# SCZwangxiao/video-ReTaKe

Measured on NVIDIA B200. Metric: 2048-frame DPSelect+PivotKV frames/s, higher is better.
Workload: dtype bf16

## Files before the change

### video-retake_b200/csrc/pivot_misc.cu

```cuda
#include <climits>

#include <stdlib.h>

#include "rtk_common.cuh"

namespace rtk {

struct RopeParams {
    int heads, L, D, n_pos, forward;
    long long stride_h, stride_l, out_stride_h, out_stride_l;
    int heads2;
    const __nv_bfloat16* x2;
    __nv_bfloat16* out2;
    long long stride_h2, stride_l2, out_stride_h2, out_stride_l2;
    int bound[6];
    float inv_scale2;
};

static bool mrope_bounds(int n_pos, const int32_t* sec, int64_t D, int bound[6]) {
    int acc = 0;
    for (int i = 0; i < 6; ++i) {
        acc += n_pos == 3 ? sec[i % 3] : 0;
        bound[i] = acc;
    }
    return n_pos != 3 || acc == D;
}

__device__ __forceinline__ int rope_pos_row(const RopeParams& p, int c) {
    if (p.n_pos == 1) return 0;
    int i = 0;
    while (i < 5 && c >= p.bound[i]) ++i;
    return i % 3;
}

__global__ void __launch_bounds__(256)
pivot_rope_table_kernel(const long long* __restrict__ pos, const float* __restrict__ inv_freq, RopeParams p, float scaling,
                        __nv_bfloat16* __restrict__ cos_t, __nv_bfloat16* __restrict__ sin_t) {
    pdl_enter();
    const int half = p.D >> 1;
    const long long total = (long long)p.L * p.D;
    for (long long i = (long long)blockIdx.x * blockDim.x + threadIdx.x; i < total; i += (long long)gridDim.x * blockDim.x) {
        const int c = (int)(i % p.D);
        const int l = (int)(i / p.D);
        const long long pv = pos[(size_t)rope_pos_row(p, c) * p.L + l];
        const float ang = inv_freq[c < half ? c : c - half] * (float)pv;
        cos_t[i] = __float2bfloat16_rn(cosf(ang) * scaling);
        sin_t[i] = __float2bfloat16_rn(sinf(ang) * scaling);
    }
}

__device__ __forceinline__ void rope_rotate_pair(float xa, float xb, float cosa, float sina, float cosb, float sinb, int forward,
                                                 float inv_scale2, __nv_bfloat16& oa, __nv_bfloat16& ob) {
    const float ta = round_bf16(xa * cosa), ra = round_bf16(-xb * sina);
    const float tb = round_bf16(xb * cosb), rb = round_bf16(xa * sinb);
    float ya, yb;
    if (forward) {
        ya = ta + ra;
        yb = tb + rb;
    } else {
        ya = round_bf16(ta - ra) * inv_scale2;
        yb = round_bf16(tb - rb) * inv_scale2;
    }
    oa = __float2bfloat16_rn(ya);
    ob = __float2bfloat16_rn(yb);
}

__device__ __forceinline__ void rope_table_entry(const RopeParams& p, const float* __restrict__ inv_freq, const long long* pv,
                                                 int c, float scaling, float& co, float& si) {
    const int half = p.D >> 1;
    const float ang = inv_freq[c < half ? c : c - half] * (float)pv[rope_pos_row(p, c)];
    co = __bfloat162float(__float2bfloat16_rn(cosf(ang) * scaling));
    si = __bfloat162float(__float2bfloat16_rn(sinf(ang) * scaling));
}

#ifndef RTK_UNROPE_TOK
#define RTK_UNROPE_TOK 2
#endif
constexpr int kUnropeTok = RTK_UNROPE_TOK;

__device__ __forceinline__ uint32_t sub_bf16x2_rn(uint32_t a, uint32_t b) {
    uint32_t d;
    asm("sub.rn.bf16x2 %0, %1, %2;" : "=r"(d) : "r"(a), "r"(b));
    return d;
}
__device__ __forceinline__ uint32_t add_bf16x2_rn(uint32_t a, uint32_t b) {
    uint32_t d;
    asm("add.rn.bf16x2 %0, %1, %2;" : "=r"(d) : "r"(a), "r"(b));
    return d;
}
__device__ __forceinline__ void unrotate_bf16x2(uint32_t xa, uint32_t xb, uint32_t cs, uint32_t sn, bool scale, float inv_scale2,
                                                uint32_t& oa, uint32_t& ob) {
    const uint32_t ta = mul_bf16x2_rn(xa, cs), ra = mul_bf16x2_rn(xb ^ 0x80008000u, sn);
    const uint32_t tb = mul_bf16x2_rn(xb, cs), rb = mul_bf16x2_rn(xa, sn);
    oa = sub_bf16x2_rn(ta, ra);
    ob = sub_bf16x2_rn(tb, rb);
    if (scale) {
        oa = scale_bf16x2_rn(oa, inv_scale2);
        ob = scale_bf16x2_rn(ob, inv_scale2);
    }
}

__device__ __forceinline__ void unrope_qk_body(const __nv_bfloat16* __restrict__ x, const long long* __restrict__ pos,
                                               const float* __restrict__ inv_freq, float scaling,
                                               __nv_bfloat16* __restrict__ out, const RopeParams& p) {
    __shared__ __align__(16) __nv_bfloat16 s_cos[kUnropeTok][128], s_sin[kUnropeTok][128];
    const int half = p.D >> 1;
    const int vec_per_row = half >> 3;
    const int ntask = (p.heads + p.heads2) * vec_per_row;
    const int tid = threadIdx.x;
    const bool scale = p.inv_scale2 != 1.0f;
    const int v0 = tid % vec_per_row, h0 = tid / vec_per_row;
    const bool second0 = h0 >= p.heads;
    const long long src_h0 = second0 ? (long long)(h0 - p.heads) * p.stride_h2 : (long long)h0 * p.stride_h;
    const long long src_l0 = second0 ? p.stride_l2 : p.stride_l;
    const __nv_bfloat16* src0 = (second0 ? p.x2 : x) + src_h0 + v0 * 8;
    for (int l0 = blockIdx.x * kUnropeTok; l0 < p.L; l0 += gridDim.x * kUnropeTok) {
        const int nl = min(kUnropeTok, p.L - l0);
        uint4 lo4[kUnropeTok], hi4[kUnropeTok];
        if (tid < ntask) {
#pragma unroll
            for (int t = 0; t < kUnropeTok; ++t) {
                if (t < nl) {
                    lo4[t] = *reinterpret_cast<const uint4*>(src0 + (l0 + t) * src_l0);
                    hi4[t] = *reinterpret_cast<const uint4*>(src0 + (l0 + t) * src_l0 + half);
                }
            }
        }
        for (int e = tid; e < nl * half; e += blockDim.x) {
            const int t = e / half, c = e - t * half;
            long long pv[3] = {0, 0, 0};
            for (int r = 0; r < p.n_pos; ++r) pv[r] = pos[(size_t)r * p.L + l0 + t];
            float co, si;
            rope_table_entry(p, inv_freq, pv, c, scaling, co, si);
            s_cos[t][c] = __float2bfloat16_rn(co);
            s_sin[t][c] = __float2bfloat16_rn(si);
        }
        __syncthreads();
#pragma unroll
        for (int t = 0; t < kUnropeTok; ++t) {
            if (t >= nl) break;
            const int l = l0 + t;
            for (int task = tid; task < ntask; task += blockDim.x) {
                const int v = task % vec_per_row, h = task / vec_per_row;
                const int c0 = v * 8;
                const bool second = h >= p.heads;
                const __nv_bfloat16* src = second ? p.x2 + (h - p.heads) * p.stride_h2 + l * p.stride_l2 : x + h * p.stride_h + l * p.stride_l;
                __nv_bfloat16* dst = second ? p.out2 + (h - p.heads) * p.out_stride_h2 + l * p.out_stride_l2
                                            : out + h * p.out_stride_h + l * p.out_stride_l;
                uint4 a4 = lo4[t], b4 = hi4[t];
                if (task != tid) {
                    a4 = *reinterpret_cast<const uint4*>(src + c0);
                    b4 = *reinterpret_cast<const uint4*>(src + c0 + half);
                }
                const uint4 cs = *reinterpret_cast<const uint4*>(&s_cos[t][c0]);
                const uint4 sn = *reinterpret_cast<const uint4*>(&s_sin[t][c0]);
                uint4 ol4, oh4;
                unrotate_bf16x2(a4.x, b4.x, cs.x, sn.x, scale, p.inv_scale2, ol4.x, oh4.x);
                unrotate_bf16x2(a4.y, b4.y, cs.y, sn.y, scale, p.inv_scale2, ol4.y, oh4.y);
                unrotate_bf16x2(a4.z, b4.z, cs.z, sn.z, scale, p.inv_scale2, ol4.z, oh4.z);
                unrotate_bf16x2(a4.w, b4.w, cs.w, sn.w, scale, p.inv_scale2, ol4.w, oh4.w);
                *reinterpret_cast<uint4*>(dst + c0) = ol4;
                *reinterpret_cast<uint4*>(dst + c0 + half) = oh4;
            }
        }
        __syncthreads();
    }
}

struct BatchLayers {
    const __nv_bfloat16* q[kMaxBatchLayers];
    const __nv_bfloat16* k[kMaxBatchLayers];
    const __nv_bfloat16* k_in[kMaxBatchLayers];
    const __nv_bfloat16* v[kMaxBatchLayers];
    __nv_bfloat16* qu[kMaxBatchLayers];
    __nv_bfloat16* ku[kMaxBatchLayers];
    const long long* pos[kMaxBatchLayers];
    const uint8_t* keymask[kMaxBatchLayers];
    __nv_bfloat16* k_out[kMaxBatchLayers];
    __nv_bfloat16* v_out[kMaxBatchLayers];
    long long* pos_out[kMaxBatchLayers];
    int32_t* keep_idx[kMaxBatchLayers];
    const __nv_bfloat16* head_scores[kMaxBatchLayers];
    long long q_stride_h[kMaxBatchLayers], q_stride_l[kMaxBatchLayers];
    long long kin_stride_h[kMaxBatchLayers], kin_stride_l[kMaxBatchLayers];
    long long k_stride_h[kMaxBatchLayers], k_stride_l[kMaxBatchLayers];
    long long v_stride_h[kMaxBatchLayers], v_stride_l[kMaxBatchLayers];
    long long out_stride_h[kMaxBatchLayers], pos_out_stride[kMaxBatchLayers];
};

__global__ void __launch_bounds__(256)
pivot_unrope_qk_batch_kernel(const __grid_constant__ BatchLayers t, const float* __restrict__ inv_freq, float scaling, RopeParams p) {
    pdl_enter();
    const int layer = blockIdx.y;
    p.stride_h = t.q_stride_h[layer]; p.stride_l = t.q_stride_l[layer];
    p.x2 = t.k_in[layer]; p.out2 = t.ku[layer];
    p.stride_h2 = t.kin_stride_h[layer]; p.stride_l2 = t.kin_stride_l[layer];
    unrope_qk_body(t.q[layer], t.pos[layer], inv_freq, scaling, t.qu[layer], p);
}

__global__ void __launch_bounds__(256)
pivot_rope_kernel(const __nv_bfloat16* __restrict__ x, const __nv_bfloat16* __restrict__ cos_t,
                  const __nv_bfloat16* __restrict__ sin_t, __nv_bfloat16* __restrict__ out, RopeParams p) {
    pdl_enter();
    const int half = p.D >> 1;
    const int vec_per_row = half >> 3;
    const long long total = (long long)(p.heads + p.heads2) * p.L * vec_per_row;
    for (long long i = (long long)blockIdx.x * blockDim.x + threadIdx.x; i < total; i += (long long)gridDim.x * blockDim.x) {
        const int v = (int)(i % vec_per_row);
        const long long hl = i / vec_per_row;
        const int l = (int)(hl % p.L);
        const int h = (int)(hl / p.L);
        const int c0 = v * 8;
        const bool second = h >= p.heads;
        const __nv_bfloat16* src = second ? p.x2 + (h - p.heads) * p.stride_h2 + l * p.stride_l2 : x + h * p.stride_h + l * p.stride_l;
        __nv_bfloat16* dst = second ? p.out2 + (h - p.heads) * p.out_stride_h2 + l * p.out_stride_l2
                                    : out + h * p.out_stride_h + l * p.out_stride_l;
        uint4 lo4 = *reinterpret_cast<const uint4*>(src + c0);
        uint4 hi4 = *reinterpret_cast<const uint4*>(src + c0 + half);
        const __nv_bfloat16* xl = reinterpret_cast<const __nv_bfloat16*>(&lo4);
        const __nv_bfloat16* xh = reinterpret_cast<const __nv_bfloat16*>(&hi4);
        uint4 ol4, oh4;
        __nv_bfloat16* ol = reinterpret_cast<__nv_bfloat16*>(&ol4);
        __nv_bfloat16* oh = reinterpret_cast<__nv_bfloat16*>(&oh4);
        const int rowa0 = rope_pos_row(p, c0), rowa1 = rope_pos_row(p, c0 + 7);
        const int rowb0 = rope_pos_row(p, c0 + half), rowb1 = rope_pos_row(p, c0 + half + 7);
        uint4 ca4, sa4, cb4, sb4;
        __nv_bfloat16* cav = reinterpret_cast<__nv_bfloat16*>(&ca4);
        __nv_bfloat16* sav = reinterpret_cast<__nv_bfloat16*>(&sa4);
        __nv_bfloat16* cbv = reinterpret_cast<__nv_bfloat16*>(&cb4);
        __nv_bfloat16* sbv = reinterpret_cast<__nv_bfloat16*>(&sb4);
        if (rowa0 == rowa1 && rowb0 == rowb1) {
            const size_t ia = ((size_t)rowa0 * p.L + l) * p.D + c0, ib = ((size_t)rowb0 * p.L + l) * p.D + c0 + half;
            ca4 = __ldg(reinterpret_cast<const uint4*>(cos_t + ia));
            sa4 = __ldg(reinterpret_cast<const uint4*>(sin_t + ia));
            cb4 = __ldg(reinterpret_cast<const uint4*>(cos_t + ib));
            sb4 = __ldg(reinterpret_cast<const uint4*>(sin_t + ib));
        } else {
#pragma unroll
            for (int e = 0; e < 8; ++e) {
                const int ca = c0 + e, cb = c0 + e + half;
                const size_t ia = ((size_t)rope_pos_row(p, ca) * p.L + l) * p.D + ca;
                const size_t ib = ((size_t)rope_pos_row(p, cb) * p.L + l) * p.D + cb;
                cav[e] = cos_t[ia]; sav[e] = sin_t[ia]; cbv[e] = cos_t[ib]; sbv[e] = sin_t[ib];
            }
        }
#pragma unroll
        for (int e = 0; e < 8; ++e)
            rope_rotate_pair(__bfloat162float(xl[e]), __bfloat162float(xh[e]), __bfloat162float(cav[e]), __bfloat162float(sav[e]),
                             __bfloat162float(cbv[e]), __bfloat162float(sbv[e]), p.forward, p.inv_scale2, ol[e], oh[e]);
        *reinterpret_cast<uint4*>(dst + c0) = ol4;
        *reinterpret_cast<uint4*>(dst + c0 + half) = oh4;
    }
}

bool key_elision_enabled();

struct KeyElide {
    const uint8_t* keymask[kMaxBatchLayers];
    int32_t* slot[kMaxBatchLayers];
    const __nv_bfloat16* k[kMaxBatchLayers];
    long long k_stride_h[kMaxBatchLayers], k_stride_l[kMaxBatchLayers];
    __nv_bfloat16* kc[kMaxBatchLayers];
    int32_t* n_keys;
    int L, KVH, D;
};

__global__ void __launch_bounds__(1024)
pivot_keymask_scan_kernel(const __grid_constant__ KeyElide e) {
    pdl_enter();
    __shared__ int wsum[32];
    const int layer = blockIdx.x, tid = threadIdx.x, lane = tid & 31, warp = tid >> 5;
    const uint8_t* __restrict__ m = e.keymask[layer];
    int32_t* __restrict__ slot = e.slot[layer];
    const int per = (e.L + 1023) / 1024;
    const int beg = min(tid * per, e.L), end = min(beg + per, e.L);
    int cnt = 0;
    for (int i = beg; i < end; ++i) cnt += !(m && m[i]);
    int inc = cnt;
#pragma unroll
    for (int o = 1; o < 32; o <<= 1) {
        const int n = __shfl_up_sync(0xffffffffu, inc, o);
        if (lane >= o) inc += n;
    }
    if (lane == 31) wsum[warp] = inc;
    __syncthreads();
    if (warp == 0) {
        const int w = wsum[lane];
        int winc = w;
#pragma unroll
        for (int o = 1; o < 32; o <<= 1) {
            const int n = __shfl_up_sync(0xffffffffu, winc, o);
            if (lane >= o) winc += n;
        }
        wsum[lane] = winc - w;
        if (lane == 31) e.n_keys[layer] = winc;
    }
    __syncthreads();
    int base = wsum[warp] + inc - cnt;
    for (int i = beg; i < end; ++i) slot[i] = (m && m[i]) ? -1 : base++;
}

__global__ void __launch_bounds__(256)
pivot_keys_compact_kernel(const __grid_constant__ KeyElide e) {
    pdl_enter();
    const int layer = blockIdx.y;
    const int vpr = e.D >> 3;
    const long long total = (long long)e.L * e.KVH * vpr;
    const int32_t* __restrict__ slot = e.slot[layer];
    for (long long i = (long long)blockIdx.x * blockDim.x + threadIdx.x; i < total; i += (long long)gridDim.x * blockDim.x) {
        const int v = (int)(i % vpr);
        const long long lh = i / vpr;
        const int h = (int)(lh % e.KVH);
        const int l = (int)(lh / e.KVH);
        const int sl = slot[l];
        if (sl < 0) continue;
        const uint4 w = __ldg(reinterpret_cast<const uint4*>(e.k[layer] + h * e.k_stride_h[layer] + l * e.k_stride_l[layer] + v * 8));
        *reinterpret_cast<uint4*>(e.kc[layer] + ((size_t)sl * e.KVH + h) * e.D + v * 8) = w;
    }
}

static int key_elide_prepare(KeyElide& ke, int n, ScoreBatch& sb, cudaStream_t st) {
    RTK_LAUNCH_PDL(pivot_keymask_scan_kernel, (unsigned)n, 1024, 0, st, ke);
    const long long total = (long long)ke.L * ke.KVH * (ke.D >> 3);
    long long gx = (total + 255) / 256;
    if (gx > 148 * 8) gx = 148 * 8;
    RTK_LAUNCH_PDL(pivot_keys_compact_kernel, dim3((unsigned)gx, (unsigned)n), 256, 0, st, ke);
    for (int i = 0; i < n; ++i) {
        sb.kc[i] = ke.kc[i];
        sb.slot[i] = ke.slot[i];
    }
    sb.n_keys = ke.n_keys;
    return 0;
}

static size_t key_elide_bytes(int64_t KVH, int64_t L, int64_t D) {
    return (((size_t)KVH * L * D * 2 + 255) & ~(size_t)255) + (((size_t)L * 4 + 255) & ~(size_t)255);
}

constexpr int kSelThreads = 1024;

__device__ void block_select_top(const uint32_t* keys, int L, int keep, int32_t* out_idx, int* sh ,
                                 int low_bit ) {
    const int tid = threadIdx.x, lane = tid & 31, warp = tid >> 5;
    const int per = (L + kSelThreads - 1) / kSelThreads;
    const int beg = min(tid * per, L), end = min(beg + per, L);
    uint32_t prefix = 0;
    for (int bit = 31; bit >= low_bit; --bit) {
        const uint32_t cand = prefix | (1u << bit);
        int cnt = 0;
        for (int i = beg; i < end; ++i) cnt += (keys[i] >= cand);
        cnt = __reduce_add_sync(0xffffffffu, cnt);
        int* buf = sh + 40 + 32 * (bit & 1);
        if (lane == 0) buf[warp] = cnt;
        __syncthreads();
        const int total = __reduce_add_sync(0xffffffffu, buf[lane]);
        if (total >= keep) prefix = cand;
    }
    __syncthreads();
    if (low_bit > 0 && (!(prefix & 0x80000000u) || (prefix >> low_bit) == (0xffffffffu >> low_bit)))
        prefix |= (1u << low_bit) - 1u;
    int gt = 0, eq = 0;
    for (int i = beg; i < end; ++i) { gt += (keys[i] > prefix); eq += (keys[i] == prefix); }
    auto block_excl_scan = [&](int v, int& total) {
        int inc = v;
#pragma unroll
        for (int o = 1; o < 32; o <<= 1) {
            const int n = __shfl_up_sync(0xffffffffu, inc, o);
            if (lane >= o) inc += n;
        }
        __syncthreads();
        if (lane == 31) sh[1 + warp] = inc;
        __syncthreads();
        if (warp == 0) {
            int w = sh[1 + lane], winc = w;
#pragma unroll
            for (int o = 1; o < 32; o <<= 1) {
                const int n = __shfl_up_sync(0xffffffffu, winc, o);
                if (lane >= o) winc += n;
            }
            sh[1 + lane] = winc - w;
            if (lane == 31) sh[33] = winc;
        }
        __syncthreads();
        total = sh[33];
        return sh[1 + warp] + inc - v;
    };
    int gt_total, eq_total;
    const int gt_before = block_excl_scan(gt, gt_total);
    const int eq_before = block_excl_scan(eq, eq_total);
    const int need = keep - gt_total;
    const int eq_taken_before = min(eq_before, need);
    int slot = gt_before + eq_taken_before;
    int eq_seen = eq_before;
    for (int i = beg; i < end; ++i) {
        const uint32_t k = keys[i];
        bool take = k > prefix;
        if (k == prefix) { take = eq_seen < need; ++eq_seen; }
        if (take) out_idx[slot++] = i;
    }
}

__device__ __forceinline__ void pivot_select_body(const __nv_bfloat16* __restrict__ head_scores, int KVH, int L,
                                                  const uint8_t* __restrict__ keymask, int keep, int32_t* __restrict__ keep_idx,
                                                  __nv_bfloat16* __restrict__ score_out, const long long* __restrict__ tpos,
                                                  long long* __restrict__ tmin_out) {
    extern __shared__ __align__(128) uint8_t smem[];
    uint32_t* keys = reinterpret_cast<uint32_t*>(smem);
    int* sh = reinterpret_cast<int*>(smem + (size_t)L * 4);
    const float rcp = 1.0f / (float)KVH;
    for (int i = threadIdx.x; i < L; i += blockDim.x) {
        float v[4] = {0.f, 0.f, 0.f, 0.f};
        for (int j = 0; j < KVH; ++j) v[j & 3] += __bfloat162float(head_scores[(size_t)j * L + i]);
        const __nv_bfloat16 s = __float2bfloat16_rn((((v[0] + v[1]) + v[2]) + v[3]) * rcp);
        if (score_out) score_out[i] = s;
        const float f = (keymask && keymask[i]) ? 1.0f : __bfloat162float(s);
        keys[i] = f32_to_ordered(f);
    }
    __syncthreads();
    block_select_top(keys, L, keep, keep_idx, sh, 16);
    if (tmin_out) {
        __syncthreads();
        long long* smin = reinterpret_cast<long long*>((reinterpret_cast<uintptr_t>(sh) + 7) & ~(uintptr_t)7);
        long long mn = LLONG_MAX;
        for (int j = threadIdx.x; j < keep; j += blockDim.x) mn = min(mn, tpos[keep_idx[j]]);
#pragma unroll
        for (int o = 16; o > 0; o >>= 1) mn = min(mn, __shfl_xor_sync(0xffffffffu, mn, o));
        if ((threadIdx.x & 31) == 0) smin[threadIdx.x >> 5] = mn;
        __syncthreads();
        if (threadIdx.x == 0) {
            for (int w = 1; w < (int)(blockDim.x >> 5); ++w) mn = min(mn, smin[w]);
            *tmin_out = mn;
        }
    }
}

__device__ __forceinline__ void st_release_sys(uint32_t* p, uint32_t v) {
    asm volatile("st.release.sys.global.u32 [%0], %1;" ::"l"(p), "r"(v) : "memory");
}
__device__ __forceinline__ uint32_t ld_acquire_sys(const uint32_t* p) {
    uint32_t v;
    asm volatile("ld.acquire.sys.global.u32 %0, [%1];" : "=r"(v) : "l"(p) : "memory");
    return v;
}
__device__ __forceinline__ unsigned long long globaltimer_ns() {
    unsigned long long t;
    asm volatile("mov.u64 %0, %%globaltimer;" : "=l"(t));
    return t;
}
__device__ __forceinline__ void xchg_wait(const uint32_t* flags, int n, uint32_t epoch, unsigned long long timeout_ns) {
    if ((int)threadIdx.x < n) {
        const unsigned long long t0 = globaltimer_ns();
        while (ld_acquire_sys(flags + threadIdx.x) != epoch) {
            __nanosleep(64);
            if (timeout_ns && globaltimer_ns() - t0 > timeout_ns) __trap();
        }
    }
    __syncthreads();
}
struct XchgPutBatch {
    const __nv_bfloat16* src[kMaxBatchLayers];
    __nv_bfloat16* dst[kMaxBatchLayers][8];
    long long n;
    int world, rank;
};
__global__ void __launch_bounds__(1024)
pivot_xchg_put_batch_kernel(const __grid_constant__ XchgPutBatch p) {
    pdl_enter();
    const int layer = blockIdx.x;
    const __nv_bfloat16* src = p.src[layer];
    for (int r = 0; r < p.world; ++r) {
        if (r == p.rank) continue;
        __nv_bfloat16* dst = p.dst[layer][r];
        if ((((uintptr_t)src | (uintptr_t)dst) & 15u) == 0) {
            const long long nv = p.n >> 3;
            for (long long i = threadIdx.x; i < nv; i += blockDim.x)
                reinterpret_cast<uint4*>(dst)[i] = reinterpret_cast<const uint4*>(src)[i];
            for (long long i = (nv << 3) + threadIdx.x; i < p.n; i += blockDim.x) dst[i] = src[i];
        } else {
            for (long long i = threadIdx.x; i < p.n; i += blockDim.x) dst[i] = src[i];
        }
    }
    __threadfence_system();
}
struct XchgFlags {
    uint32_t* flags[8];
    int world, rank;
    uint32_t epoch;
};
__global__ void __launch_bounds__(32)
pivot_xchg_flag_kernel(XchgFlags p) {
    pdl_enter();
    __threadfence_system();
    if ((int)threadIdx.x < p.world) st_release_sys(p.flags[threadIdx.x] + p.rank, p.epoch);
}

__global__ void __launch_bounds__(kSelThreads)
pivot_select_kernel(const __nv_bfloat16* __restrict__ head_scores, int KVH, int L, const uint8_t* __restrict__ keymask,
                    int keep, int32_t* __restrict__ keep_idx, __nv_bfloat16* __restrict__ score_out) {
    pdl_enter();
    pivot_select_body(head_scores, KVH, L, keymask, keep, keep_idx, score_out, nullptr, nullptr);
}

__global__ void __launch_bounds__(kSelThreads)
pivot_select_batch_kernel(const __grid_constant__ BatchLayers t, int KVH, int L, int keep, int reforge, long long* __restrict__ tmin,
                          const uint32_t* __restrict__ wait_flags, int wait_n, uint32_t wait_epoch, unsigned long long wait_ns) {
    pdl_enter();
    if (wait_flags) xchg_wait(wait_flags, wait_n, wait_epoch, wait_ns);
    const int layer = blockIdx.x;
    pivot_select_body(t.head_scores[layer], KVH, L, t.keymask[layer], keep, t.keep_idx[layer], nullptr,
                      reforge ? t.pos[layer] : nullptr, reforge ? tmin + layer : nullptr);
}

struct CompactParams {
    int KVH, L, D, keep, n_pos, reforge;
    long long stride_h, stride_l, out_stride_h;
    long long v_stride_h, v_stride_l;
    long long pos_out_stride;
    float ratio;
};

__global__ void __launch_bounds__(256)
pivot_compact_kernel(const __nv_bfloat16* __restrict__ k, const __nv_bfloat16* __restrict__ v,
                     const int32_t* __restrict__ keep_idx, __nv_bfloat16* __restrict__ k_out,
                     __nv_bfloat16* __restrict__ v_out, const long long* __restrict__ pos,
                     long long* __restrict__ pos_out, CompactParams p) {
    pdl_enter();
    if (blockIdx.x == gridDim.x - 1) {
        if (!pos) return;
        __shared__ long long smin[32];
        const int tid = threadIdx.x, lane = tid & 31, warp = tid >> 5;
        for (int r = p.reforge ? 1 : 0; r < p.n_pos; ++r)
            for (int j = tid; j < p.keep; j += blockDim.x) pos_out[(size_t)r * p.keep + j] = pos[(size_t)r * p.L + keep_idx[j]];
        if (!p.reforge) return;
        long long mn = LLONG_MAX;
        for (int j = tid; j < p.keep; j += blockDim.x) mn = min(mn, pos[keep_idx[j]]);
#pragma unroll
        for (int o = 16; o > 0; o >>= 1) mn = min(mn, __shfl_xor_sync(0xffffffffu, mn, o));
        if (lane == 0) smin[warp] = mn;
        __syncthreads();
        mn = smin[0];
        for (int w = 1; w < (int)(blockDim.x >> 5); ++w) mn = min(mn, smin[w]);
        for (int j = tid; j < p.keep; j += blockDim.x) {
            const float d = (float)(pos[keep_idx[j]] - mn);
            pos_out[j] = mn + (long long)(d * p.ratio);
        }
        return;
    }
    const int vec_per_row = p.D >> 3;
    const long long total = (long long)p.KVH * p.keep * vec_per_row;
    const long long nthreads = (long long)(gridDim.x - 1) * blockDim.x;
    for (long long i = (long long)blockIdx.x * blockDim.x + threadIdx.x; i < total; i += nthreads) {
        const int c = (int)(i % vec_per_row);
        const long long hj = i / vec_per_row;
        const int j = (int)(hj % p.keep);
        const int h = (int)(hj / p.keep);
        const int src_row = keep_idx[j];
        const size_t so = (size_t)h * p.stride_h + (size_t)src_row * p.stride_l + (size_t)c * 8;
        const size_t sv = (size_t)h * p.v_stride_h + (size_t)src_row * p.v_stride_l + (size_t)c * 8;
        const size_t dof = (size_t)h * p.out_stride_h + (size_t)j * p.D + (size_t)c * 8;
        if (k) *reinterpret_cast<uint4*>(k_out + dof) = __ldg(reinterpret_cast<const uint4*>(k + so));
        if (v) *reinterpret_cast<uint4*>(v_out + dof) = __ldg(reinterpret_cast<const uint4*>(v + sv));
    }
}

__device__ __forceinline__ void compact_rope_body(const __nv_bfloat16* __restrict__ k, const __nv_bfloat16* __restrict__ v,
                                                  const int32_t* __restrict__ keep_idx, __nv_bfloat16* __restrict__ k_out,
                                                  __nv_bfloat16* __restrict__ v_out, const long long* __restrict__ pos,
                                                  long long* __restrict__ pos_out, const long long* __restrict__ tmin,
                                                  const float* __restrict__ inv_freq, float scaling, const CompactParams& p,
                                                  const RopeParams& rp, int rotate) {
    __shared__ float s_cos[256], s_sin[256];
    __shared__ long long s_pos[3];
    const int j = blockIdx.x, tid = threadIdx.x;
    const int src_row = keep_idx[j];
    if (pos && tid < p.n_pos) {
        long long pv = pos[(size_t)tid * p.L + src_row];
        if (p.reforge && tid == 0) {
            const long long mn = *tmin;
            pv = mn + (long long)((float)(pv - mn) * p.ratio);
        }
        pos_out[(size_t)tid * p.pos_out_stride + j] = pv;
        s_pos[tid] = pv;
    }
    const int vec_per_row = p.D >> 3;
    for (int t = tid; t < p.KVH * vec_per_row; t += blockDim.x) {
        const int c = t % vec_per_row, h = t / vec_per_row;
        const size_t dof = (size_t)h * p.out_stride_h + (size_t)j * p.D + (size_t)c * 8;
        *reinterpret_cast<uint4*>(v_out + dof) =
            __ldg(reinterpret_cast<const uint4*>(v + (size_t)h * p.v_stride_h + (size_t)src_row * p.v_stride_l + (size_t)c * 8));
        if (!rotate)
            *reinterpret_cast<uint4*>(k_out + dof) =
                __ldg(reinterpret_cast<const uint4*>(k + (size_t)h * p.stride_h + (size_t)src_row * p.stride_l + (size_t)c * 8));
    }
    if (!rotate) return;
    __syncthreads();
    if (tid < p.D) rope_table_entry(rp, inv_freq, s_pos, tid, scaling, s_cos[tid], s_sin[tid]);
    __syncthreads();
    const int half = p.D >> 1, hv = half >> 3;
    for (int t = tid; t < p.KVH * hv; t += blockDim.x) {
        const int c0 = (t % hv) * 8, h = t / hv;
        const __nv_bfloat16* src = k + (size_t)h * p.stride_h + (size_t)src_row * p.stride_l;
        __nv_bfloat16* dst = k_out + (size_t)h * p.out_stride_h + (size_t)j * p.D;
        uint4 lo4 = *reinterpret_cast<const uint4*>(src + c0);
        uint4 hi4 = *reinterpret_cast<const uint4*>(src + c0 + half);
        const __nv_bfloat16* xl = reinterpret_cast<const __nv_bfloat16*>(&lo4);
        const __nv_bfloat16* xh = reinterpret_cast<const __nv_bfloat16*>(&hi4);
        uint4 ol4, oh4;
        __nv_bfloat16* ol = reinterpret_cast<__nv_bfloat16*>(&ol4);
        __nv_bfloat16* oh = reinterpret_cast<__nv_bfloat16*>(&oh4);
#pragma unroll
        for (int e = 0; e < 8; ++e)
            rope_rotate_pair(__bfloat162float(xl[e]), __bfloat162float(xh[e]), s_cos[c0 + e], s_sin[c0 + e], s_cos[c0 + half + e],
                             s_sin[c0 + half + e], 1, 1.0f, ol[e], oh[e]);
        *reinterpret_cast<uint4*>(dst + c0) = ol4;
        *reinterpret_cast<uint4*>(dst + c0 + half) = oh4;
    }
}

__global__ void __launch_bounds__(128)
pivot_compact_rope_batch_kernel(const __grid_constant__ BatchLayers t, const long long* __restrict__ tmin,
                                const float* __restrict__ inv_freq, float scaling, CompactParams p, RopeParams rp, int rotate) {
    pdl_enter();
    const int layer = blockIdx.y;
    p.stride_h = t.k_stride_h[layer]; p.stride_l = t.k_stride_l[layer];
    p.v_stride_h = t.v_stride_h[layer]; p.v_stride_l = t.v_stride_l[layer];
    p.out_stride_h = t.out_stride_h[layer];
    p.pos_out_stride = t.pos_out_stride[layer];
    compact_rope_body(t.k[layer], t.v[layer], t.keep_idx[layer], t.k_out[layer], t.v_out[layer], t.pos[layer], t.pos_out[layer],
                      tmin + layer, inv_freq, scaling, p, rp, rotate);
}

struct CopyJobs {
    int n;
    const __nv_bfloat16* src[4];
    __nv_bfloat16* dst[4];
    int heads[4], rows[4];
    long long src_stride_h[4], src_stride_l[4], dst_stride_h[4], dst_stride_l[4];
    long long vec_end[4];
    int D;
};

__global__ void __launch_bounds__(256)
kv_block_copy_kernel(CopyJobs j) {
    pdl_enter();
    const int vpr = j.D >> 3;
    const long long total = j.vec_end[j.n - 1];
    for (long long i = (long long)blockIdx.x * blockDim.x + threadIdx.x; i < total; i += (long long)gridDim.x * blockDim.x) {
        int k = 0;
        while (i >= j.vec_end[k]) ++k;
        const long long li = i - (k ? j.vec_end[k - 1] : 0);
        const int c = (int)(li % vpr);
        const long long hr = li / vpr;
        const int r = (int)(hr % j.rows[k]);
        const int h = (int)(hr / j.rows[k]);
        const uint4 v = __ldg(reinterpret_cast<const uint4*>(j.src[k] + h * j.src_stride_h[k] + r * j.src_stride_l[k] + c * 8));
        *reinterpret_cast<uint4*>(j.dst[k] + h * j.dst_stride_h[k] + r * j.dst_stride_l[k] + c * 8) = v;
    }
}

long long g_launches = 0;
static int g_key_elision = -1;
bool key_elision_enabled() {
    if (g_key_elision < 0) {
        const char* e = getenv("RTK_NO_KEY_ELISION");
        g_key_elision = (e && e[0] == '1') ? 0 : 1;
    }
    return g_key_elision != 0;
}
unsigned long long xchg_timeout_ns() {
    static const unsigned long long ns = [] {
        const char* e = getenv("RTK_XCHG_TIMEOUT_S");
        const double s = (e && e[0]) ? atof(e) : 120.0;
        return s > 0.0 ? (unsigned long long)(s * 1e9) : 0ull;
    }();
    return ns;
}
bool pdl_enabled() {
    static const bool on = [] {
        const char* e = getenv("RTK_NO_PDL");
        return !(e && e[0] && e[0] != '0');
    }();
    return on;
}

}

using namespace rtk;

extern "C" int rtk_version(void) { return RTK_ABI_VERSION; }

extern "C" int rtk_debug_key_elision(int on) {
    const int prev = rtk::key_elision_enabled() ? 1 : 0;
    if (on >= 0) rtk::g_key_elision = on ? 1 : 0;
    return prev;
}

#ifndef RTK_BUILD_ID
#define RTK_BUILD_ID "unknown"
#endif
extern "C" const char* rtk_build_id(void) { return RTK_BUILD_ID; }

extern "C" int64_t rtk_launch_count(void) { return (int64_t)rtk::g_launches; }

extern "C" const char* rtk_error_string(int code) {
    if (code == 0) return "ok";
    if (code > 0) return cudaGetErrorString((cudaError_t)code);
    switch (code) {
        case RTK_E_BADARG: return "rtk: bad argument (null pointer or non-positive size)";
        case RTK_E_ALIGN: return "rtk: pointer or stride not 16-byte aligned";
        case RTK_E_UNSUPPORTED: return "rtk: shape outside the supported envelope";
        case RTK_E_WORKSPACE: return "rtk: workspace too small";
        case RTK_E_DRIVER: return "rtk: cuTensorMapEncodeTiled unavailable or failed";
        default: return "rtk: unknown error";
    }
}

static int rope_launch(const void* x, const void* cos, const void* sin, void* out, const RopeParams& p, cudaStream_t st) {
    const long long total = (long long)(p.heads + p.heads2) * p.L * (p.D / 16);
    long long grid = (total + 255) / 256;
    if (grid > 148 * 16) grid = 148 * 16;
    RTK_LAUNCH_PDL(pivot_rope_kernel, (unsigned)grid, 256, 0, st, (const __nv_bfloat16*)x, (const __nv_bfloat16*)cos, (const __nv_bfloat16*)sin, (__nv_bfloat16*)out, p);
    return 0;
}

extern "C" int rtk_pivot_rope(const void* x, int64_t heads, int64_t L, int64_t D, int64_t stride_h, int64_t stride_l,
                              const void* cos, const void* sin, int n_pos, const int32_t* mrope_section_host,
                              float inv_scale2, int forward, void* out, int64_t out_stride_h, int64_t out_stride_l,
                              void* stream) {
    RTK_NVTX("rtk_pivot_rope");
    if (!x || !cos || !sin || !out || heads < 1 || L < 1 || D < 16) return RTK_E_BADARG;
    if (D % 16 != 0 || (n_pos != 1 && n_pos != 3)) return RTK_E_UNSUPPORTED;
    if (n_pos == 3 && !mrope_section_host) return RTK_E_BADARG;
    if ((((uintptr_t)x | (uintptr_t)out) & 15u) != 0) return RTK_E_ALIGN;
    if ((stride_h | stride_l | out_stride_h | out_stride_l) % 8 != 0) return RTK_E_ALIGN;
    RopeParams p;
    p.heads = (int)heads; p.L = (int)L; p.D = (int)D; p.n_pos = n_pos; p.forward = forward;
    p.stride_h = stride_h; p.stride_l = stride_l; p.out_stride_h = out_stride_h; p.out_stride_l = out_stride_l;
    p.inv_scale2 = inv_scale2;
    p.heads2 = 0; p.x2 = nullptr; p.out2 = nullptr;
    p.stride_h2 = p.stride_l2 = p.out_stride_h2 = p.out_stride_l2 = 0;
    if (!mrope_bounds(n_pos, mrope_section_host, D, p.bound)) return RTK_E_UNSUPPORTED;
    return rope_launch(x, cos, sin, out, p, (cudaStream_t)stream);
}

extern "C" int rtk_pivot_select(const void* head_scores, int64_t KVH, int64_t L, const uint8_t* keymask, int64_t keep,
                                int32_t* keep_idx, void* score_out, void* stream) {
    RTK_NVTX("rtk_pivot_select");
    if (!head_scores || !keep_idx || KVH < 1 || L < 1 || keep < 1 || keep > L) return RTK_E_BADARG;
    if (L > 16384) return RTK_E_UNSUPPORTED;
    const size_t smem = (size_t)L * 4 + 112 * 4;
    cudaError_t e = cudaFuncSetAttribute(pivot_select_kernel, cudaFuncAttributeMaxDynamicSharedMemorySize, (int)smem);
    if (e != cudaSuccess) return (int)e;
    RTK_LAUNCH_PDL(pivot_select_kernel, 1, kSelThreads, smem, (cudaStream_t)stream, (const __nv_bfloat16*)head_scores, (int)KVH,
                   (int)L, keymask, (int)keep, keep_idx, (__nv_bfloat16*)score_out);
    return 0;
}

extern "C" int rtk_pivot_compact(const void* k, const void* v, int64_t KVH, int64_t L, int64_t D, int64_t stride_h,
                                 int64_t stride_l, const int32_t* keep_idx, int64_t keep, void* k_out, void* v_out,
                                 int64_t out_stride_h, const int64_t* pos, int n_pos, int64_t* pos_out, int reforge,
                                 void* stream) {
    RTK_NVTX("rtk_pivot_compact");
    if ((!k && !v) || !keep_idx || (k && !k_out) || (v && !v_out) || KVH < 1 || L < 1 || D < 8 || keep < 1 || keep > L)
        return RTK_E_BADARG;
    if (pos && (!pos_out || n_pos < 1)) return RTK_E_BADARG;
    if (D % 8 != 0) return RTK_E_UNSUPPORTED;
    if ((((uintptr_t)k | (uintptr_t)v | (uintptr_t)k_out | (uintptr_t)v_out) & 15u) != 0) return RTK_E_ALIGN;
    if ((stride_h | stride_l | out_stride_h) % 8 != 0) return RTK_E_ALIGN;
    CompactParams p;
    p.KVH = (int)KVH; p.L = (int)L; p.D = (int)D; p.keep = (int)keep; p.n_pos = n_pos; p.reforge = reforge;
    p.stride_h = stride_h; p.stride_l = stride_l; p.out_stride_h = out_stride_h;
    p.v_stride_h = stride_h; p.v_stride_l = stride_l;
    p.pos_out_stride = keep;
    p.ratio = (float)((double)keep / (double)L);
    const long long total = KVH * keep * (D / 8);
    long long grid = (total + 255) / 256;
    if (grid > 148 * 8) grid = 148 * 8;
    RTK_LAUNCH_PDL(pivot_compact_kernel, (unsigned)(grid + 1), 256, 0, (cudaStream_t)stream,  (const __nv_bfloat16*)k, (const __nv_bfloat16*)v, keep_idx, (__nv_bfloat16*)k_out, (__nv_bfloat16*)v_out, (const long long*)pos, (long long*)pos_out, p);
    return 0;
}

extern "C" int rtk_pivot_rope_tables(const int64_t* pos, int n_pos, int64_t L, int64_t D, const float* inv_freq,
                                     const int32_t* mrope_section_host, float attention_scaling, void* cos_out,
                                     void* sin_out, void* stream) {
    RTK_NVTX("rtk_pivot_rope_tables");
    if (!pos || !inv_freq || !cos_out || !sin_out || L < 1 || D < 2) return RTK_E_BADARG;
    if (D % 2 != 0 || (n_pos != 1 && n_pos != 3)) return RTK_E_UNSUPPORTED;
    if (n_pos == 3 && !mrope_section_host) return RTK_E_BADARG;
    RopeParams p;
    p.heads = 1; p.L = (int)L; p.D = (int)D; p.n_pos = n_pos; p.forward = 0;
    p.stride_h = p.stride_l = p.out_stride_h = p.out_stride_l = 0;
    p.heads2 = 0; p.x2 = nullptr; p.out2 = nullptr;
    p.stride_h2 = p.stride_l2 = p.out_stride_h2 = p.out_stride_l2 = 0;
    p.inv_scale2 = 1.0f;
    if (!mrope_bounds(n_pos, mrope_section_host, D, p.bound)) return RTK_E_UNSUPPORTED;
    long long grid = (L * D + 255) / 256;
    if (grid > 148 * 8) grid = 148 * 8;
    RTK_LAUNCH_PDL(pivot_rope_table_kernel, (unsigned)grid, 256, 0, (cudaStream_t)stream,  (const long long*)pos, inv_freq, p, attention_scaling, (__nv_bfloat16*)cos_out, (__nv_bfloat16*)sin_out);
    return 0;
}

static size_t align256(size_t x) { return (x + 255) & ~(size_t)255; }

extern "C" size_t rtk_pivot_update_batch_workspace_bytes(int64_t H, int64_t KVH, int64_t L, int64_t D, int64_t n_layers) {
    if (H < 1 || KVH < 1 || L < 1 || D < 1 || n_layers < 1) return 0;
    const size_t n = (size_t)(n_layers < kMaxBatchLayers ? n_layers : kMaxBatchLayers);
    return align256(rtk_pivot_score_workspace_bytes(H * (int64_t)n, L)) +
           n * (align256((size_t)H * L * D * 2) + align256((size_t)KVH * L * D * 2)) + align256(n * sizeof(long long)) + 256 +
           n * key_elide_bytes(KVH, L, D) + 256;
}

extern "C" size_t rtk_pivot_update_workspace_bytes(int64_t H, int64_t KVH, int64_t L, int64_t D) {
    return rtk_pivot_update_batch_workspace_bytes(H, KVH, L, D, 1);
}

#ifndef RTK_UNROT_TOKEN_MAJOR
#define RTK_UNROT_TOKEN_MAJOR 1
#endif

static int pivot_update_group(const rtk_pivot_update_args* a, int n, char* ws, cudaStream_t st) {
    const rtk_pivot_update_args& a0 = a[0];
    const int64_t H = a0.H, KVH = a0.KVH, L = a0.L, D = a0.D;
    const bool reforge = a0.reforge != 0;
    const int64_t uq_sh = RTK_UNROT_TOKEN_MAJOR ? D : L * D, uq_sl = RTK_UNROT_TOKEN_MAJOR ? H * D : D;
    const int64_t uk_sh = RTK_UNROT_TOKEN_MAJOR ? D : L * D, uk_sl = RTK_UNROT_TOKEN_MAJOR ? KVH * D : D;
    void* score_ws = ws;                ws += align256(rtk_pivot_score_workspace_bytes(H * n, L));
    char* qu0 = ws;                     ws += (size_t)n * align256((size_t)H * L * D * 2);
    char* ku0 = ws;                     ws += (size_t)n * align256((size_t)KVH * L * D * 2);
    long long* tmin = (long long*)ws;   ws += align256((size_t)n * sizeof(long long)) + 256;
    char* kc0 = ws;                     ws += (size_t)n * align256((size_t)KVH * L * D * 2);
    char* slot0 = ws;                   ws += (size_t)n * align256((size_t)L * 4);
    int32_t* nkeys_ws = (int32_t*)ws;

    BatchLayers t = {};
    ScoreBatch sb = {};
    sb.n = n; sb.H = H; sb.KVH = KVH; sb.L = L; sb.D = D;
    for (int i = 0; i < kMaxBatchLayers; ++i) {
        const rtk_pivot_update_args& x = a[i < n ? i : 0];
        char* qu = qu0 + (size_t)(i < n ? i : 0) * align256((size_t)H * L * D * 2);
        char* ku = ku0 + (size_t)(i < n ? i : 0) * align256((size_t)KVH * L * D * 2);
        t.q[i] = (const __nv_bfloat16*)x.q;       t.q_stride_h[i] = x.q_stride_h;     t.q_stride_l[i] = x.q_stride_l;
        t.k_in[i] = (const __nv_bfloat16*)x.k;    t.kin_stride_h[i] = x.k_stride_h;   t.kin_stride_l[i] = x.k_stride_l;
        t.qu[i] = (__nv_bfloat16*)qu;             t.ku[i] = (__nv_bfloat16*)ku;
        t.k[i] = reforge ? (const __nv_bfloat16*)ku : (const __nv_bfloat16*)x.k;
        t.k_stride_h[i] = reforge ? uk_sh : x.k_stride_h;
        t.k_stride_l[i] = reforge ? uk_sl : x.k_stride_l;
        t.v[i] = (const __nv_bfloat16*)x.v;       t.v_stride_h[i] = x.v_stride_h;     t.v_stride_l[i] = x.v_stride_l;
        t.pos[i] = (const long long*)x.pos;       t.keymask[i] = x.keymask;
        t.k_out[i] = (__nv_bfloat16*)x.k_out;     t.v_out[i] = (__nv_bfloat16*)x.v_out;
        t.out_stride_h[i] = x.out_stride_h;
        t.pos_out[i] = (long long*)x.pos_out;     t.pos_out_stride[i] = x.pos_out_stride > 0 ? x.pos_out_stride : x.keep;
        t.keep_idx[i] = x.keep_idx;               t.head_scores[i] = (const __nv_bfloat16*)x.head_scores;
        if (i < n) {
            sb.q[i] = reforge ? (const void*)qu : x.q;
            sb.k[i] = reforge ? (const void*)ku : x.k;
            sb.q_stride_h[i] = reforge ? uq_sh : x.q_stride_h;   sb.q_stride_l[i] = reforge ? uq_sl : x.q_stride_l;
            sb.k_stride_h[i] = reforge ? uk_sh : x.k_stride_h;   sb.k_stride_l[i] = reforge ? uk_sl : x.k_stride_l;
            sb.head_scores[i] = x.head_scores;
        }
    }
    RopeParams rp = {};
    rp.heads = (int)H; rp.L = (int)L; rp.D = (int)D; rp.n_pos = a0.n_pos; rp.forward = 0;
    rp.out_stride_h = uq_sh; rp.out_stride_l = uq_sl;
    rp.heads2 = (int)KVH; rp.out_stride_h2 = uk_sh; rp.out_stride_l2 = uk_sl;
    rp.inv_scale2 = a0.inv_scale2;
    mrope_bounds(a0.n_pos, a0.mrope_section, D, rp.bound);
    const bool xchg = a0.xchg_world > 1;
    const int64_t score_rows = a0.score_rows > 0 ? a0.score_rows : KVH;
    if (reforge && !a0.skip_score) {
        if (a0.inv_freq) {
            RTK_LAUNCH_PDL(pivot_unrope_qk_batch_kernel, dim3((unsigned)((L + kUnropeTok - 1) / kUnropeTok), (unsigned)n), 256, 0, st, t, a0.inv_freq,
                           a0.attention_scaling, rp);
        } else {
            rp.stride_h = a0.q_stride_h; rp.stride_l = a0.q_stride_l;
            rp.x2 = t.k_in[0]; rp.out2 = t.ku[0]; rp.stride_h2 = a0.k_stride_h; rp.stride_l2 = a0.k_stride_l;
            const int rc = rope_launch(a0.q, a0.cos, a0.sin, t.qu[0], rp, st);
            if (rc) return rc;
        }
    }
    if (!a0.skip_score) {
        bool any_mask = false;
        for (int i = 0; i < n; ++i) any_mask = any_mask || a[i].keymask != nullptr;
        if (any_mask && key_elision_enabled()) {
            KeyElide ke = {};
            ke.L = (int)L; ke.KVH = (int)KVH; ke.D = (int)D; ke.n_keys = nkeys_ws;
            for (int i = 0; i < kMaxBatchLayers; ++i) {
                const int j = i < n ? i : 0;
                ke.keymask[i] = a[j].keymask;
                ke.slot[i] = (int32_t*)(slot0 + (size_t)j * align256((size_t)L * 4));
                ke.k[i] = t.k[j]; ke.k_stride_h[i] = t.k_stride_h[j]; ke.k_stride_l[i] = t.k_stride_l[j];
                ke.kc[i] = (__nv_bfloat16*)(kc0 + (size_t)j * align256((size_t)KVH * L * D * 2));
            }
            int rc = key_elide_prepare(ke, n, sb, st);
            if (rc) return rc;
        }
        if (a0.ev_score_begin) cudaEventRecord((cudaEvent_t)a0.ev_score_begin, st);
        int rc = pivot_score_batch(sb, score_ws, rtk_pivot_score_workspace_bytes(H * n, L), st);
        if (rc) return rc;
        if (a0.ev_score_end) cudaEventRecord((cudaEvent_t)a0.ev_score_end, st);
    }
    if (a0.skip_select) {
        if (xchg) {
            XchgPutBatch xp = {};
            xp.n = (long long)KVH * L; xp.world = a0.xchg_world; xp.rank = a0.xchg_rank;
            for (int i = 0; i < n; ++i) {
                xp.src[i] = (const __nv_bfloat16*)a[i].head_scores;
                for (int r = 0; r < a0.xchg_world; ++r)
                    xp.dst[i][r] = (__nv_bfloat16*)a[i].xchg_scores[r] + (size_t)a0.xchg_rank * KVH * L;
            }
            RTK_LAUNCH_PDL(pivot_xchg_put_batch_kernel, (unsigned)n, 1024, 0, st, xp);
            XchgFlags xf = {};
            xf.world = a0.xchg_world; xf.rank = a0.xchg_rank; xf.epoch = a0.xchg_epoch;
            for (int r = 0; r < a0.xchg_world; ++r) xf.flags[r] = a0.xchg_flags[r];
            RTK_LAUNCH_PDL(pivot_xchg_flag_kernel, 1, 32, 0, st, xf);
        }
        return 0;
    }
    {
        const size_t smem = (size_t)L * 4 + 112 * 4;
        cudaError_t e = cudaFuncSetAttribute(pivot_select_batch_kernel, cudaFuncAttributeMaxDynamicSharedMemorySize, (int)smem);
        if (e != cudaSuccess) return (int)e;
        RTK_LAUNCH_PDL(pivot_select_batch_kernel, (unsigned)n, kSelThreads, smem, st, t, (int)score_rows, (int)L, (int)a0.keep,
                       reforge ? 1 : 0, tmin, (const uint32_t*)(xchg ? a0.xchg_flags[a0.xchg_rank] : nullptr),
                       xchg ? a0.xchg_world : 0, a0.xchg_epoch, xchg_timeout_ns());
    }
    {
        CompactParams p = {};
        p.KVH = (int)KVH; p.L = (int)L; p.D = (int)D; p.keep = (int)a0.keep; p.n_pos = a0.pos ? a0.n_pos : 0; p.reforge = a0.reforge;
        p.ratio = (float)((double)a0.keep / (double)L);
        RopeParams rq = {};
        rq.D = (int)D; rq.n_pos = a0.n_pos; rq.L = (int)a0.keep;
        for (int i = 0; i < 6; ++i) rq.bound[i] = rp.bound[i];
        RTK_LAUNCH_PDL(pivot_compact_rope_batch_kernel, dim3((unsigned)a0.keep, (unsigned)n), 128, 0, st, t, (const long long*)tmin,
                       a0.inv_freq, a0.attention_scaling, p, rq, (reforge && a0.inv_freq) ? 1 : 0);
    }
    return 0;
}

static int update_check(const rtk_pivot_update_args* layers, int64_t n, const void* workspace, size_t workspace_bytes) {
    if (!layers || n < 1 || !workspace) return RTK_E_BADARG;
    const rtk_pivot_update_args& a0 = layers[0];
    const bool scores = !a0.skip_score, selects = !a0.skip_select, xchg = a0.xchg_world > 1;
    if (!scores && !selects) return RTK_E_BADARG;
    if (a0.H < 1 || a0.KVH < 1 || a0.L < 1 || (selects && (a0.keep < 1 || a0.keep > a0.L))) return RTK_E_BADARG;
    if (a0.L > 16384 || a0.D % 16 != 0 || a0.D > 256) return RTK_E_UNSUPPORTED;
    if (scores && ((a0.D != 64 && a0.D != 128) || a0.H % a0.KVH != 0 || a0.H > 256)) return RTK_E_UNSUPPORTED;
    if (xchg) {
        if (n > kMaxBatchLayers) return RTK_E_UNSUPPORTED;
        if (a0.xchg_world > 8 || a0.xchg_rank < 0 || a0.xchg_rank >= a0.xchg_world || (scores && selects)) return RTK_E_BADARG;
    }
    if (a0.reforge && !a0.inv_freq && n > 1) return RTK_E_UNSUPPORTED;
    int bound[6];
    if (a0.reforge && (scores || a0.inv_freq) && !mrope_bounds(a0.n_pos, a0.mrope_section, a0.D, bound)) return RTK_E_UNSUPPORTED;
    if (((uintptr_t)workspace & 255u) != 0) return RTK_E_ALIGN;
    if (workspace_bytes < rtk_pivot_update_batch_workspace_bytes(a0.H, a0.KVH, a0.L, a0.D, n)) return RTK_E_WORKSPACE;
    for (int64_t i = 0; i < n; ++i) {
        const rtk_pivot_update_args& x = layers[i];
        if (!x.q || !x.k || !x.v || !x.k_out || !x.v_out || !x.keep_idx || !x.head_scores) return RTK_E_BADARG;
        if (x.H != a0.H || x.KVH != a0.KVH || x.L != a0.L || x.D != a0.D || x.keep != a0.keep || x.reforge != a0.reforge ||
            x.n_pos != a0.n_pos || x.inv_freq != a0.inv_freq || x.attention_scaling != a0.attention_scaling ||
            x.inv_scale2 != a0.inv_scale2 || x.skip_select != a0.skip_select || x.skip_score != a0.skip_score ||
            x.score_rows != a0.score_rows || x.xchg_world != a0.xchg_world || x.xchg_rank != a0.xchg_rank ||
            x.xchg_epoch != a0.xchg_epoch || (x.pos == nullptr) != (a0.pos == nullptr))
            return RTK_E_UNSUPPORTED;
        for (int j = 0; j < 3; ++j)
            if (x.mrope_section[j] != a0.mrope_section[j]) return RTK_E_UNSUPPORTED;
        if (x.reforge && (!x.pos || !x.pos_out || (!x.inv_freq && (!x.cos || !x.sin)))) return RTK_E_BADARG;
        if (xchg) {
            for (int r = 0; r < a0.xchg_world; ++r)
                if (!x.xchg_scores[r] || !a0.xchg_flags[r]) return RTK_E_BADARG;
            const char* own = (const char*)x.xchg_scores[a0.xchg_rank];
            if (a0.skip_score && (const char*)x.head_scores != own) return RTK_E_BADARG;
            if (a0.skip_select && (const char*)x.head_scores != own + (size_t)a0.xchg_rank * a0.KVH * a0.L * 2) return RTK_E_BADARG;
        }
        if (x.pos && (selects || x.reforge) && (!x.pos_out || x.n_pos < 1 || x.n_pos > 3)) return RTK_E_BADARG;
        uintptr_t ptrs = 0;
        int64_t strides = 0;
        if (scores) {
            ptrs |= (uintptr_t)x.q;
            strides |= x.q_stride_h | x.q_stride_l;
        }
        if (scores || !x.reforge) {
            ptrs |= (uintptr_t)x.k;
            strides |= x.k_stride_h | x.k_stride_l;
        }
        if (selects) {
            ptrs |= (uintptr_t)x.v | (uintptr_t)x.k_out | (uintptr_t)x.v_out;
            strides |= x.v_stride_h | x.v_stride_l | x.out_stride_h;
        }
        if ((ptrs & 15u) != 0 || strides % 8 != 0) return RTK_E_ALIGN;
    }
    return 0;
}

extern "C" int rtk_pivot_update(const rtk_pivot_update_args* a, void* stream) {
    RTK_NVTX("rtk_pivot_update");
    if (!a) return RTK_E_BADARG;
    const int rc = update_check(a, 1, a->workspace, a->workspace_bytes);
    if (rc) return rc;
    return pivot_update_group(a, 1, (char*)a->workspace, (cudaStream_t)stream);
}

extern "C" int rtk_pivot_update_batch(const rtk_pivot_update_args* layers, int64_t n_layers, void* workspace,
                                      size_t workspace_bytes, void* stream) {
    RTK_NVTX("rtk_pivot_update_batch");
    int rc = update_check(layers, n_layers, workspace, workspace_bytes);
    if (rc) return rc;
    for (int64_t i = 0; i < n_layers; i += kMaxBatchLayers) {
        const int n = (int)((n_layers - i) < kMaxBatchLayers ? (n_layers - i) : kMaxBatchLayers);
        rc = pivot_update_group(layers + i, n, (char*)workspace, (cudaStream_t)stream);
        if (rc) return rc;
    }
    return 0;
}

extern "C" int rtk_kv_block_copy(int n_jobs, const void* const* src, void* const* dst, const int64_t* heads, const int64_t* rows,
                                 const int64_t* src_stride_h, const int64_t* src_stride_l, const int64_t* dst_stride_h,
                                 const int64_t* dst_stride_l, int64_t D, void* stream) {
    RTK_NVTX("rtk_kv_block_copy");
    if (n_jobs < 1 || n_jobs > 4 || !src || !dst || !heads || !rows || D < 8) return RTK_E_BADARG;
    if (D % 8 != 0) return RTK_E_UNSUPPORTED;
    CopyJobs j;
    j.n = n_jobs;
    j.D = (int)D;
    long long acc = 0;
    for (int k = 0; k < n_jobs; ++k) {
        if (!src[k] || !dst[k] || heads[k] < 1 || rows[k] < 0) return RTK_E_BADARG;
        if ((((uintptr_t)src[k] | (uintptr_t)dst[k]) & 15u) != 0) return RTK_E_ALIGN;
        if ((src_stride_h[k] | src_stride_l[k] | dst_stride_h[k] | dst_stride_l[k]) % 8 != 0) return RTK_E_ALIGN;
        j.src[k] = (const __nv_bfloat16*)src[k];
        j.dst[k] = (__nv_bfloat16*)dst[k];
        j.heads[k] = (int)heads[k];
        j.rows[k] = (int)rows[k];
        j.src_stride_h[k] = src_stride_h[k]; j.src_stride_l[k] = src_stride_l[k];
        j.dst_stride_h[k] = dst_stride_h[k]; j.dst_stride_l[k] = dst_stride_l[k];
        acc += heads[k] * rows[k] * (D / 8);
        j.vec_end[k] = acc;
    }
    for (int k = n_jobs; k < 4; ++k) j.vec_end[k] = acc;
    if (acc == 0) return 0;
    long long grid = (acc + 255) / 256;
    if (grid > 148 * 8) grid = 148 * 8;
    RTK_LAUNCH_PDL(kv_block_copy_kernel, (unsigned)grid, 256, 0, (cudaStream_t)stream, j);
    return 0;
}
```

### video-retake_b200/csrc/pivot_score.cu

```cuda
#include <cuda.h>

#include "rtk_common.cuh"

namespace rtk {

constexpr int kTile = 128;
constexpr int kHeadDim = 128;
constexpr int kPair = 2;
constexpr int kStages = 2;
constexpr int kASlots = 2;
constexpr int kAccBufs = 4;
constexpr int kStatSlots = kStages + kAccBufs;
constexpr uint32_t kTileBytes = kTile * kHeadDim * 2;
constexpr uint32_t kHalfBytes = kTile * 64 * 2;

struct ScoreSmem {
    static constexpr uint32_t a_tile = 0;
    static constexpr uint32_t b_ring = kASlots * kPair * kTileBytes;
    static constexpr uint32_t stats = b_ring + kStages * kTileBytes;
    static constexpr uint32_t merge = stats + kStatSlots * kTile * 4;
    static constexpr uint32_t bars = merge + 4 * kTile * 2 * 4;
    static constexpr uint32_t n_bars = 4 + 2 * kStages + 2 * kAccBufs + kStatSlots;
    static constexpr uint32_t tmem_ptr = bars + n_bars * 8;
    static constexpr uint32_t total = tmem_ptr + 16;
};

__device__ __forceinline__ void tmem_alloc(uint32_t smem_dst, uint32_t ncols) {
    asm volatile("tcgen05.alloc.cta_group::1.sync.aligned.shared::cta.b32 [%0], %1;" ::"r"(smem_dst), "r"(ncols) : "memory");
    asm volatile("tcgen05.relinquish_alloc_permit.cta_group::1.sync.aligned;" ::: "memory");
}
__device__ __forceinline__ void tmem_dealloc(uint32_t taddr, uint32_t ncols) {
    asm volatile("tcgen05.dealloc.cta_group::1.sync.aligned.b32 %0, %1;" ::"r"(taddr), "r"(ncols) : "memory");
}
__device__ __forceinline__ void tc_fence_before() { asm volatile("tcgen05.fence::before_thread_sync;" ::: "memory"); }
__device__ __forceinline__ void tc_fence_after() { asm volatile("tcgen05.fence::after_thread_sync;" ::: "memory"); }
__device__ __forceinline__ void tc_commit(uint32_t bar) {
    asm volatile("tcgen05.commit.cta_group::1.mbarrier::arrive::one.shared::cluster.b64 [%0];" ::"r"(bar) : "memory");
}
__device__ __forceinline__ void umma_bf16(uint32_t tmem_d, uint64_t adesc, uint64_t bdesc, uint32_t idesc, uint32_t accum) {
    asm volatile(
        "{\n\t.reg .pred p;\n\t"
        "setp.ne.b32 p, %4, 0;\n\t"
        "tcgen05.mma.cta_group::1.kind::f16 [%0], %1, %2, %3, p;\n\t}"
        ::"r"(tmem_d), "l"(adesc), "l"(bdesc), "r"(idesc), "r"(accum)
        : "memory");
}
__device__ __forceinline__ void tmem_ld_wait() { asm volatile("tcgen05.wait::ld.sync.aligned;" ::: "memory"); }
__device__ __forceinline__ void tmem_ld64(uint32_t taddr, uint32_t (&r)[64]) {
    asm volatile(
        "tcgen05.ld.sync.aligned.32x32b.x64.b32 "
        "{%0, %1, %2, %3, %4, %5, %6, %7, %8, %9, %10, %11, %12, %13, %14, %15, "
        "%16, %17, %18, %19, %20, %21, %22, %23, %24, %25, %26, %27, %28, %29, %30, %31, "
        "%32, %33, %34, %35, %36, %37, %38, %39, %40, %41, %42, %43, %44, %45, %46, %47, "
        "%48, %49, %50, %51, %52, %53, %54, %55, %56, %57, %58, %59, %60, %61, %62, %63}, [%64];"
        : "=r"(r[0]), "=r"(r[1]), "=r"(r[2]), "=r"(r[3]), "=r"(r[4]), "=r"(r[5]), "=r"(r[6]), "=r"(r[7]),
          "=r"(r[8]), "=r"(r[9]), "=r"(r[10]), "=r"(r[11]), "=r"(r[12]), "=r"(r[13]), "=r"(r[14]), "=r"(r[15]),
          "=r"(r[16]), "=r"(r[17]), "=r"(r[18]), "=r"(r[19]), "=r"(r[20]), "=r"(r[21]), "=r"(r[22]), "=r"(r[23]),
          "=r"(r[24]), "=r"(r[25]), "=r"(r[26]), "=r"(r[27]), "=r"(r[28]), "=r"(r[29]), "=r"(r[30]), "=r"(r[31]),
          "=r"(r[32]), "=r"(r[33]), "=r"(r[34]), "=r"(r[35]), "=r"(r[36]), "=r"(r[37]), "=r"(r[38]), "=r"(r[39]),
          "=r"(r[40]), "=r"(r[41]), "=r"(r[42]), "=r"(r[43]), "=r"(r[44]), "=r"(r[45]), "=r"(r[46]), "=r"(r[47]),
          "=r"(r[48]), "=r"(r[49]), "=r"(r[50]), "=r"(r[51]), "=r"(r[52]), "=r"(r[53]), "=r"(r[54]), "=r"(r[55]),
          "=r"(r[56]), "=r"(r[57]), "=r"(r[58]), "=r"(r[59]), "=r"(r[60]), "=r"(r[61]), "=r"(r[62]), "=r"(r[63])
        : "r"(taddr)
        : "memory");
}
__device__ __forceinline__ void add_bf16_pair(float& acc_lo, float& acc_hi, uint32_t packed) {
    asm("{\n\t.reg .b16 lo, hi;\n\t"
        "mov.b32 {lo, hi}, %2;\n\t"
        "add.rn.f32.bf16 %0, lo, %0;\n\t"
        "add.rn.f32.bf16 %1, hi, %1;\n\t}"
        : "+f"(acc_lo), "+f"(acc_hi)
        : "r"(packed));
}

__device__ __forceinline__ void tma_load_3d(uint32_t dst, const CUtensorMap* map, int c0, int c1, int c2, uint32_t bar) {
    asm volatile(
        "cp.async.bulk.tensor.3d.shared::cluster.global.tile.mbarrier::complete_tx::bytes [%0], [%1, {%3, %4, %5}], [%2];"
        ::"r"(dst), "l"(reinterpret_cast<uint64_t>(map)), "r"(bar), "r"(c0), "r"(c1), "r"(c2)
        : "memory");
}
__device__ __forceinline__ float ex2f(float x) {
    float y;
    asm("ex2.approx.ftz.f32 %0, %1;" : "=f"(y) : "f"(x));
    return y;
}
__device__ __forceinline__ float lg2f(float x) {
    float y;
    asm("lg2.approx.ftz.f32 %0, %1;" : "=f"(y) : "f"(x));
    return y;
}

__device__ __forceinline__ uint64_t umma_desc_sw128(uint32_t smem_addr) {
    return (uint64_t)((smem_addr & 0x3ffffu) >> 4) | ((uint64_t)1 << 16) | ((uint64_t)(1024 >> 4) << 32) |
           ((uint64_t)1 << 46) | ((uint64_t)2 << 61);
}
constexpr uint32_t kIdesc = (1u << 4) | (1u << 7) | (1u << 10) | ((uint32_t)(kTile >> 3) << 17) | ((uint32_t)(kTile >> 4) << 24);

template <int NL>
struct ScoreMaps {
    CUtensorMap q[NL], k[NL];
    CUtensorMap kc[NL];
};

struct ScoreParams {
    int H, G, L, nt;
    int Hl;
    int n_atoms;
    int q_dim1_is_l, k_dim1_is_l;
    float inv_sqrt_d;
    const int32_t* n_keys;
    int kc_dim1_is_l;
    float2* ml_part;
    float* stats;
    float* colsum_part;
};

constexpr float kLog2e = 1.4426950408889634f;

__device__ __forceinline__ uint64_t pk2(float lo, float hi) {
    uint64_t d;
    asm("mov.b64 %0, {%1, %2};" : "=l"(d) : "f"(lo), "f"(hi));
    return d;
}
__device__ __forceinline__ void upk2(uint64_t v, float& lo, float& hi) {
    asm("mov.b64 {%0, %1}, %2;" : "=f"(lo), "=f"(hi) : "l"(v));
}
__device__ __forceinline__ uint64_t mul2(uint64_t a, uint64_t b) {
    uint64_t d;
    asm("mul.rn.f32x2 %0, %1, %2;" : "=l"(d) : "l"(a), "l"(b));
    return d;
}
__device__ __forceinline__ uint64_t fma2(uint64_t a, uint64_t b, uint64_t c) {
    uint64_t d;
    asm("fma.rn.f32x2 %0, %1, %2, %3;" : "=l"(d) : "l"(a), "l"(b), "l"(c));
    return d;
}
__device__ __forceinline__ uint64_t add2(uint64_t a, uint64_t b) {
    uint64_t d;
    asm("add.rn.f32x2 %0, %1, %2;" : "=l"(d) : "l"(a), "l"(b));
    return d;
}

__device__ __forceinline__ void mbar_wait_feeder(uint32_t bar, uint32_t parity) {
    while (!mbar_try_wait(bar, parity)) {
    }
}

__device__ __forceinline__ float round_bf16_inplace(float a) {
    uint32_t d;
    asm("cvt.rn.bf16x2.f32 %0, %1, %2;" : "=r"(d) : "f"(a), "f"(0.f));
    return __uint_as_float(d);
}

__device__ __forceinline__ uint64_t logit_chain2(uint32_t r0, uint32_t r1, uint64_t inv2) {
    float t0, t1;
    upk2(mul2(pk2(round_bf16_inplace(__uint_as_float(r0)), round_bf16_inplace(__uint_as_float(r1))), inv2), t0, t1);
    return pk2(round_bf16_inplace(t0), round_bf16_inplace(t1));
}
__device__ __forceinline__ float logit_chain1(float acc, float inv) { return round_bf16(round_bf16(acc) * inv); }

__device__ __forceinline__ uint64_t ex2_mufu2(uint64_t x2) {
    float x0, x1;
    upk2(x2, x0, x1);
    return pk2(ex2f(x0), ex2f(x1));
}

struct SoftmaxState {
    float m = -INFINITY;
    uint64_t acc = 0;
    float c0 = 0.f, c1 = 0.f;
};

template <int PASS>
__device__ __forceinline__ void softmax_cols(uint32_t (&r)[64], int valid, SoftmaxState& st, const float* cq, float inv,
                                             uint64_t inv2, uint64_t l2e2) {
    constexpr int NC = 64;
    if (PASS == 1) {
        if (valid < NC) {
#pragma unroll
            for (int i = 0; i < NC; ++i)
                if (i >= valid) r[i] = 0xff800000u;
        }
        float mx = fmaxf(fmaxf(__uint_as_float(r[0]), __uint_as_float(r[1])), __uint_as_float(r[2]));
#pragma unroll
        for (int i = 3; i < NC - 1; i += 2) mx = fmaxf(fmaxf(mx, __uint_as_float(r[i])), __uint_as_float(r[i + 1]));
        mx = fmaxf(mx, __uint_as_float(r[NC - 1]));
        const float mn = fmaxf(st.m, logit_chain1(mx, inv));
        if (!(mn > -INFINITY)) return;
        const float mm = mn * kLog2e;
        const float sc = ex2f(fmaf(st.m, kLog2e, -mm));
        st.acc = mul2(st.acc, pk2(sc, sc));
        st.m = mn;
        const uint64_t nmm = pk2(-mm, -mm);
#pragma unroll
        for (int i = 0; i < NC; i += 4) {
            st.acc = add2(st.acc, ex2_mufu2(fma2(logit_chain2(r[i], r[i + 1], inv2), l2e2, nmm)));
            st.acc = add2(st.acc, ex2_mufu2(fma2(logit_chain2(r[i + 2], r[i + 3], inv2), l2e2, nmm)));
        }
    } else {
#pragma unroll
        for (int i = 0; i < NC; i += 4) {
            const float4 cc = *reinterpret_cast<const float4*>(cq + i);
            float e0, e1, e2, e3;
            upk2(ex2_mufu2(fma2(logit_chain2(r[i], r[i + 1], inv2), l2e2, pk2(-cc.x, -cc.y))), e0, e1);
            upk2(ex2_mufu2(fma2(logit_chain2(r[i + 2], r[i + 3], inv2), l2e2, pk2(-cc.z, -cc.w))), e2, e3);
            add_bf16_pair(st.c0, st.c1, pack_bf16x2_rn(e0, e1));
            add_bf16_pair(st.c0, st.c1, pack_bf16x2_rn(e2, e3));
        }
    }
}

struct TileRange {
    int g, g1, Gl;
    int nt;
    int nt_a, nta;
    int layer, n_layers, Hl, geff;
    const int32_t* n_keys;
    __device__ __forceinline__ void set_layer_range() {
        nt_a = n_keys ? (n_keys[layer] + kTile - 1) / kTile : nt;
        nta = (nt_a + kPair - 1) / kPair;
        Gl = Hl * nta * nt;
        int ge = Gl / ((nt + 1) / 2);
        ge = ge < 1 ? 1 : (ge > (int)gridDim.x ? (int)gridDim.x : ge);
        geff = ge;
        if ((int)blockIdx.x < geff) {
            g = (int)((unsigned)Gl * blockIdx.x / (unsigned)geff);
            g1 = (int)((unsigned)Gl * (blockIdx.x + 1) / (unsigned)geff);
        } else {
            g = g1 = 0;
        }
    }
    __device__ __forceinline__ bool next_cta_reaches_end_of(int ul) const {
        return (int)((unsigned)Gl * (blockIdx.x + 2) / (unsigned)geff) >= (ul + 1) * nt;
    }
    __device__ __forceinline__ TileRange(int H, int Hl_, int nt_, const int32_t* n_keys_) : nt(nt_), layer(0), Hl(Hl_), n_keys(n_keys_) {
        n_layers = H / Hl_;
        set_layer_range();
    }
    __device__ __forceinline__ bool next(int& ul, int& tb0, int& tb1) {
        while (g >= g1) {
            if (++layer >= n_layers) return false;
            set_layer_range();
        }
        ul = g / nt;
        tb0 = g - ul * nt;
        const int left = g1 - g;
        tb1 = (left < nt - tb0) ? tb0 + left : nt;
        g += tb1 - tb0;
        return true;
    }
};

constexpr int kGroups = 4;
constexpr int kSoftmaxWarps = 4 * kGroups;
constexpr int kScoreThreads2 = (2 + kSoftmaxWarps) * 32;
constexpr int kTileArrivals = 8;

template <int PASS, int NL>
__global__ void __launch_bounds__(kScoreThreads2, 1)
pivot_score_kernel(const __grid_constant__ ScoreMaps<NL> maps, ScoreParams prm) {
    if (RTK_PDL_EARLY_SCORE) pdl_trigger();
    extern __shared__ __align__(1024) uint8_t smem_raw[];
    const uint32_t base = (smem_u32(smem_raw) + 1023u) & ~1023u;
    uint8_t* smem = smem_raw + (base - smem_u32(smem_raw));
    const int warp = threadIdx.x >> 5, lane = threadIdx.x & 31;

    const uint32_t bar0 = base + ScoreSmem::bars;
    auto a_full = [&](int i) { return bar0 + 8 * i; };
    auto a_empty = [&](int i) { return bar0 + 16 + 8 * i; };
    auto b_full = [&](int s) { return bar0 + 32 + 8 * s; };
    auto b_empty = [&](int s) { return bar0 + 32 + 8 * (kStages + s); };
    auto t_full = [&](int b) { return bar0 + 32 + 8 * (2 * kStages + b); };
    auto t_empty = [&](int b) { return bar0 + 32 + 8 * (2 * kStages + kAccBufs + b); };
    auto st_full = [&](int i) { return bar0 + 32 + 8 * (2 * kStages + 2 * kAccBufs + i); };

    if (threadIdx.x == 0) {
        for (int i = 0; i < 2; ++i) { mbar_init(a_full(i), 1); mbar_init(a_empty(i), 1); }
        for (int s = 0; s < kStages; ++s) { mbar_init(b_full(s), 1); mbar_init(b_empty(s), 1); }
        for (int b = 0; b < kAccBufs; ++b) { mbar_init(t_full(b), 1); mbar_init(t_empty(b), kTileArrivals); }
        for (int i = 0; i < kStatSlots; ++i) mbar_init(st_full(i), 1);
        fence_mbar_init();
    }
    if (warp == 1) tmem_alloc(base + ScoreSmem::tmem_ptr, 512);
    tc_fence_before();
    __syncthreads();
    tc_fence_after();
    pdl_wait();
    const uint32_t tmem_base = *reinterpret_cast<volatile uint32_t*>(smem + ScoreSmem::tmem_ptr);

    const int nt = prm.nt;
    const size_t hl = (size_t)prm.H * nt * kTile;
    const bool elide = (PASS == 2) && prm.n_keys != nullptr;
    const CUtensorMap* a_maps = (PASS == 1) ? maps.q : (elide ? maps.kc : maps.k);
    const CUtensorMap* b_maps = (PASS == 1) ? maps.k : maps.q;
    const int a_l1 = (PASS == 1) ? prm.q_dim1_is_l : (elide ? prm.kc_dim1_is_l : prm.k_dim1_is_l);
    const int b_l1 = (PASS == 1) ? prm.k_dim1_is_l : prm.q_dim1_is_l;
    TileRange range(prm.H, prm.Hl, nt, elide ? prm.n_keys : nullptr);
    int ul, tb0, tb1;

    if (warp == 0) {
        if (lane == 0) {
            uint32_t cnt = 0, ucnt = 0;
            while (range.next(ul, tb0, tb1)) {
                const int layer = range.layer;
                const int h = ul / range.nta, ta = (ul - h * range.nta) * kPair;
                const int hh = layer * prm.Hl + h;
                const int nt_a = range.nt_a;
                const CUtensorMap* a_map = a_maps + layer;
                const CUtensorMap* b_map = b_maps + layer;
                const int a_head = (PASS == 1) ? h : h / prm.G;
                const int b_head = (PASS == 1) ? h / prm.G : h;
                const int as = ucnt % kASlots;
                mbar_wait_feeder(a_empty(as), ((ucnt / kASlots) & 1u) ^ 1u);
                mbar_arrive_expect_tx(a_full(as), kPair * prm.n_atoms * kHalfBytes);
                for (int pa = 0; pa < kPair; ++pa)
                    for (int kk = 0; kk < prm.n_atoms; ++kk) {
                        const int row = ((ta + pa < nt_a) ? ta + pa : ta) * kTile;
                        tma_load_3d(base + ScoreSmem::a_tile + (as * kPair + pa) * kTileBytes + kk * kHalfBytes, a_map, kk * 64,
                                    a_l1 ? row : a_head, a_l1 ? a_head : row, a_full(as));
                    }
                ++ucnt;
                for (int tb = tb0; tb < tb1; ++tb, ++cnt) {
                    const int s = cnt % kStages;
                    mbar_wait_feeder(b_empty(s), ((cnt / kStages) & 1u) ^ 1u);
                    mbar_arrive_expect_tx(b_full(s), prm.n_atoms * kHalfBytes);
                    const uint32_t dst = base + ScoreSmem::b_ring + s * kTileBytes;
                    for (int kk = 0; kk < prm.n_atoms; ++kk) {
                        const int row = tb * kTile;
                        tma_load_3d(dst + kk * kHalfBytes, b_map, kk * 64, b_l1 ? row : b_head, b_l1 ? b_head : row,
                                    b_full(s));
                    }
                    if (PASS == 2) {
                        const int sl = cnt % kStatSlots;
                        mbar_arrive_expect_tx(st_full(sl), kTile * 4u);
                        bulk_g2s(base + ScoreSmem::stats + sl * kTile * 4u,
                                 prm.stats + (size_t)hh * nt * kTile + (size_t)tb * kTile, kTile * 4u, st_full(sl));
                    }
                }
            }
        }
    } else if (warp == 1) {
        uint32_t cnt = 0, ucnt = 0;
        while (range.next(ul, tb0, tb1)) {
            const int as = ucnt % kASlots;
            mbar_wait_feeder(a_full(as), (ucnt / kASlots) & 1u);
            ++ucnt;
            for (int tb = tb0; tb < tb1; ++tb, ++cnt) {
                const int s = cnt % kStages, bp = 2 * (int)(cnt & 1u);
                mbar_wait_feeder(b_full(s), (cnt / kStages) & 1u);
                mbar_wait_feeder(t_empty(bp), ((cnt >> 1) & 1u) ^ 1u);
                mbar_wait_feeder(t_empty(bp + 1), ((cnt >> 1) & 1u) ^ 1u);
                tc_fence_after();
                if (elect_one()) {
                    const uint32_t b0 = base + ScoreSmem::b_ring + s * kTileBytes;
                    const int nks = prm.n_atoms * 4;
#pragma unroll
                    for (int pa = 0; pa < 2; ++pa) {
                        const uint32_t a0 = base + ScoreSmem::a_tile + (as * 2 + pa) * kTileBytes;
#pragma unroll 8
                        for (int ks = 0; ks < nks; ++ks) {
                            const uint32_t off = (ks >> 2) * kHalfBytes + (ks & 3) * 32;
                            umma_bf16(tmem_base + (bp + pa) * kTile, umma_desc_sw128(a0 + off), umma_desc_sw128(b0 + off), kIdesc,
                                      ks > 0 ? 1u : 0u);
                        }
                        tc_commit(t_full(bp + pa));
                    }
                    tc_commit(b_empty(s));
                    if (tb == tb1 - 1) tc_commit(a_empty(as));
                }
                __syncwarp();
            }
        }
    } else {
        const int sw = warp - 2;
        const int grp = sw >> 2;
        const int quarter = warp & 3;
        const int row = quarter * 32 + lane;
        const int half = grp & 1;
        const uint32_t lane_addr = tmem_base + ((uint32_t)(quarter * 32) << 16) + half * 64;
        float* merge = reinterpret_cast<float*>(smem + ScoreSmem::merge);
        const float inv = prm.inv_sqrt_d;
        const uint64_t inv2 = pk2(inv, inv), l2e2 = pk2(kLog2e, kLog2e);
        uint32_t cnt = 0;
        while (range.next(ul, tb0, tb1)) {
            const int hl_ = ul / range.nta, ta = (ul - hl_ * range.nta) * 2 + (grp >> 1);
            const int h = range.layer * prm.Hl + hl_;
            const bool has_tile = ta < range.nt_a;
            SoftmaxState st;
            for (int tb = tb0; tb < tb1; ++tb, ++cnt) {
                const int b = 2 * (int)(cnt & 1u) + (grp >> 1);
                mbar_wait(t_full(b), (cnt >> 1) & 1u);
                tc_fence_after();
                if (PASS == 2) mbar_wait(st_full(cnt % kStatSlots), (cnt / kStatSlots) & 1u);
                const int valid = prm.L - tb * kTile - half * 64;
                const float* cq = reinterpret_cast<const float*>(smem + ScoreSmem::stats) + (cnt % kStatSlots) * kTile + half * 64;
                if (has_tile) {
                    uint32_t r[64];
                    tmem_ld64(lane_addr + b * kTile, r);
                    tmem_ld_wait();
                    softmax_cols<PASS>(r, valid, st, cq, inv, inv2, l2e2);
                }
                tc_fence_before();
                __syncwarp();
                if (lane == 0) mbar_arrive(t_empty(b));
            }
            const float m = st.m;
            float a0, a1;
            upk2(st.acc, a0, a1);
            if (PASS == 2) { a0 = st.c0; a1 = st.c1; }
            const bool first = (tb0 == 0), last = (tb1 == nt);
            const int part = first ? 0 : (last ? 2 : 1);
            const bool fill1 = first && (last || range.next_cta_reaches_end_of(ul)), fill2 = first && last;
            const size_t o = (size_t)h * nt * kTile + (size_t)ta * kTile + row;
            const int g_lo = grp & ~1;
            const bool folder = (grp == g_lo) && has_tile;
            if (PASS == 1) {
                merge[(grp * kTile + row) * 2] = m;
                merge[(grp * kTile + row) * 2 + 1] = a0 + a1;
                asm volatile("bar.sync 1, %0;" ::"n"(kSoftmaxWarps * 32) : "memory");
                if (folder) {
                    float mn = -INFINITY;
                    for (int g = g_lo; g < g_lo + 2; ++g) mn = fmaxf(mn, merge[(g * kTile + row) * 2]);
                    float lt = 0.f;
                    for (int g = g_lo; g < g_lo + 2; ++g) {
                        const float mg = merge[(g * kTile + row) * 2];
                        if (mg > -INFINITY) lt += merge[(g * kTile + row) * 2 + 1] * ex2f((mg - mn) * kLog2e);
                    }
                    prm.ml_part[(size_t)part * hl + o] = make_float2(mn, lt);
                    if (fill1) prm.ml_part[hl + o] = make_float2(-INFINITY, 0.f);
                    if (fill2) prm.ml_part[2 * hl + o] = make_float2(-INFINITY, 0.f);
                }
                asm volatile("bar.sync 1, %0;" ::"n"(kSoftmaxWarps * 32) : "memory");
            } else {
                merge[grp * kTile + row] = a0 + a1;
                asm volatile("bar.sync 1, %0;" ::"n"(kSoftmaxWarps * 32) : "memory");
                if (folder) {
                    const float cs = merge[g_lo * kTile + row] + merge[(g_lo + 1) * kTile + row];
                    prm.colsum_part[(size_t)part * hl + o] = cs;
                    if (fill1) prm.colsum_part[hl + o] = 0.f;
                    if (fill2) prm.colsum_part[2 * hl + o] = 0.f;
                }
                asm volatile("bar.sync 1, %0;" ::"n"(kSoftmaxWarps * 32) : "memory");
            }
        }
    }
    tc_fence_before();
    __syncthreads();
    if (warp == 1) tmem_dealloc(tmem_base, 512);
}

__global__ void pivot_stats_merge_kernel(const float2* __restrict__ ml_part, int H, int L, int Lpad, float* __restrict__ stats) {
    pdl_enter();
    const int q = blockIdx.x * blockDim.x + threadIdx.x;
    const int h = blockIdx.y;
    if (q >= Lpad) return;
    const size_t o = (size_t)h * Lpad + q, hl = (size_t)H * Lpad;
    const float2 p0 = ml_part[o], p1 = ml_part[hl + o], p2 = ml_part[2 * hl + o];
    const float mn = fmaxf(fmaxf(p0.x, p1.x), p2.x);
    float lt = 0.f;
    if (p0.x > -INFINITY) lt += p0.y * ex2f((p0.x - mn) * kLog2e);
    if (p1.x > -INFINITY) lt += p1.y * ex2f((p1.x - mn) * kLog2e);
    if (p2.x > -INFINITY) lt += p2.y * ex2f((p2.x - mn) * kLog2e);
    stats[o] = (q < L) ? fmaf(mn, kLog2e, lg2f(lt)) : INFINITY;
}

struct HeadScoreOut {
    __nv_bfloat16* p[kMaxBatchLayers];
    const int32_t* slot[kMaxBatchLayers];
    int KVH;
};

__global__ void pivot_head_reduce_kernel(const float* __restrict__ colsum_part, int H, int G, int L, int Lpad,
                                         const __grid_constant__ HeadScoreOut out) {
    pdl_enter();
    const int k = blockIdx.x * blockDim.x + threadIdx.x;
    const int g = blockIdx.y;
    if (k >= L) return;
    const size_t hl = (size_t)H * Lpad;
    const int layer = g / out.KVH;
    int col = k;
    if (out.slot[layer]) {
        col = out.slot[layer][k];
        if (col < 0) {
            out.p[layer][(size_t)(g - layer * out.KVH) * L + k] = __float2bfloat16_rn(1.0f);
            return;
        }
    }
    float v[4] = {0.f, 0.f, 0.f, 0.f};
    for (int j = 0; j < G; ++j) {
        const size_t o = (size_t)(g * G + j) * Lpad + col;
        v[j & 3] += round_bf16((colsum_part[o] + colsum_part[hl + o]) + colsum_part[2 * hl + o]);
    }
    const float s = ((v[0] + v[1]) + v[2]) + v[3];
    out.p[layer][(size_t)(g - layer * out.KVH) * L + k] = __float2bfloat16_rn(s * (1.0f / (float)G));
}

typedef CUresult (*EncodeTiledFn)(CUtensorMap*, CUtensorMapDataType, cuuint32_t, void*, const cuuint64_t*, const cuuint64_t*,
                                  const cuuint32_t*, const cuuint32_t*, CUtensorMapInterleave, CUtensorMapSwizzle,
                                  CUtensorMapL2promotion, CUtensorMapFloatOOBfill);

static EncodeTiledFn get_encode_fn() {
    static EncodeTiledFn fn = nullptr;
    if (fn) return fn;
    void* p = nullptr;
    cudaDriverEntryPointQueryResult qres;
    if (cudaGetDriverEntryPoint("cuTensorMapEncodeTiled", &p, cudaEnableDefault, &qres) != cudaSuccess ||
        qres != cudaDriverEntryPointSuccess)
        return nullptr;
    fn = reinterpret_cast<EncodeTiledFn>(p);
    return fn;
}

static int make_map(CUtensorMap* map, const void* ptr, int64_t heads, int64_t L, int64_t D, int64_t stride_h,
                    int64_t stride_l, int* dim1_is_l) {
    EncodeTiledFn enc = get_encode_fn();
    if (!enc) return RTK_E_DRIVER;
    const bool l_first = (heads == 1) || (stride_l <= stride_h);
    *dim1_is_l = l_first ? 1 : 0;
    cuuint64_t dims[3] = {(cuuint64_t)D, (cuuint64_t)(l_first ? L : heads), (cuuint64_t)(l_first ? heads : L)};
    cuuint64_t strides[2] = {(cuuint64_t)((l_first ? stride_l : stride_h) * 2), (cuuint64_t)((l_first ? stride_h : stride_l) * 2)};
    if (heads == 1) strides[1] = (cuuint64_t)(stride_l * 2) * (cuuint64_t)L;
    cuuint32_t box[3] = {64u, (cuuint32_t)(l_first ? kTile : 1), (cuuint32_t)(l_first ? 1 : kTile)};
    cuuint32_t estr[3] = {1u, 1u, 1u};
    CUresult r = enc(map, CU_TENSOR_MAP_DATA_TYPE_BFLOAT16, 3, const_cast<void*>(ptr), dims, strides, box, estr,
                     CU_TENSOR_MAP_INTERLEAVE_NONE, CU_TENSOR_MAP_SWIZZLE_128B, CU_TENSOR_MAP_L2_PROMOTION_L2_256B,
                     CU_TENSOR_MAP_FLOAT_OOB_FILL_NONE);
    return r == CUDA_SUCCESS ? 0 : RTK_E_DRIVER;
}

}

using namespace rtk;

extern "C" size_t rtk_pivot_score_workspace_bytes(int64_t H, int64_t L) {
    if (H < 1 || L < 1) return 0;
    const size_t lpad = (size_t)((L + kTile - 1) / kTile) * kTile;
    return 10 * (size_t)H * lpad * sizeof(float);
}

namespace rtk {

template <int NL>
static int score_launch(const ScoreBatch& b, ScoreParams prm, cudaStream_t st) {
    ScoreMaps<NL> maps;
    for (int l = 0; l < b.n; ++l) {
        int ql = 0, kl = 0;
        int rc = make_map(&maps.q[l], b.q[l], b.H, b.L, b.D, b.q_stride_h[l], b.q_stride_l[l], &ql);
        if (rc) return rc;
        rc = make_map(&maps.k[l], b.k[l], b.KVH, b.L, b.D, b.k_stride_h[l], b.k_stride_l[l], &kl);
        if (rc) return rc;
        if (l == 0) { prm.q_dim1_is_l = ql; prm.k_dim1_is_l = kl; }
        else if (ql != prm.q_dim1_is_l || kl != prm.k_dim1_is_l) return RTK_E_UNSUPPORTED;
        if (prm.n_keys) {
            int cl = 0;
            rc = make_map(&maps.kc[l], b.kc[l], b.KVH, b.L, b.D, b.D, b.KVH * b.D, &cl);
            if (rc) return rc;
            prm.kc_dim1_is_l = cl;
        } else {
            maps.kc[l] = maps.k[l];
        }
    }
    for (int l = b.n; l < NL; ++l) { maps.q[l] = maps.q[0]; maps.k[l] = maps.k[0]; maps.kc[l] = maps.kc[0]; }
    int dev = 0, sms = 0;
    cudaGetDevice(&dev);
    cudaDeviceGetAttribute(&sms, cudaDevAttrMultiProcessorCount, dev);
    const int units = prm.Hl * ((prm.nt + kPair - 1) / kPair);
    const long long gmax = (long long)units * prm.nt / ((prm.nt + 1) / 2);
    const int grid = (int)(gmax < sms ? (gmax < 1 ? 1 : gmax) : sms);
    const size_t smem = ScoreSmem::total + 1024;
    cudaError_t e = cudaFuncSetAttribute(pivot_score_kernel<1, NL>, cudaFuncAttributeMaxDynamicSharedMemorySize, (int)smem);
    if (e != cudaSuccess) return (int)e;
    e = cudaFuncSetAttribute(pivot_score_kernel<2, NL>, cudaFuncAttributeMaxDynamicSharedMemorySize, (int)smem);
    if (e != cudaSuccess) return (int)e;
    HeadScoreOut out;
    out.KVH = (int)b.KVH;
    for (int l = 0; l < kMaxBatchLayers; ++l) {
        out.p[l] = reinterpret_cast<__nv_bfloat16*>(b.head_scores[l < b.n ? l : 0]);
        out.slot[l] = prm.n_keys ? b.slot[l < b.n ? l : 0] : nullptr;
    }
    RTK_LAUNCH_PDL((pivot_score_kernel<1, NL>), grid, kScoreThreads2, smem, st, maps, prm);
    dim3 g1((unsigned)((prm.nt * kTile + 255) / 256), (unsigned)prm.H);
    RTK_LAUNCH_PDL(pivot_stats_merge_kernel, g1, 256, 0, st, prm.ml_part, prm.H, prm.L, prm.nt * kTile, prm.stats);
    RTK_LAUNCH_PDL((pivot_score_kernel<2, NL>), grid, kScoreThreads2, smem, st, maps, prm);
    dim3 g2((unsigned)((prm.L + 255) / 256), (unsigned)(b.KVH * b.n));
    RTK_LAUNCH_PDL(pivot_head_reduce_kernel, g2, 256, 0, st, prm.colsum_part, prm.H, prm.G, prm.L, prm.nt * kTile, out);
    return 0;
}

int pivot_score_batch(const ScoreBatch& b, void* workspace, size_t workspace_bytes, cudaStream_t st) {
    if (b.n < 1 || b.n > kMaxBatchLayers || !workspace || b.H < 1 || b.KVH < 1 || b.L < 1) return RTK_E_BADARG;
    if ((b.D != 64 && b.D != 128) || b.H % b.KVH != 0 || b.L > 16384 || b.H > 256) return RTK_E_UNSUPPORTED;
    if (((uintptr_t)workspace & 15u) != 0) return RTK_E_ALIGN;
    for (int l = 0; l < b.n; ++l) {
        if (!b.q[l] || !b.k[l] || !b.head_scores[l]) return RTK_E_BADARG;
        if ((((uintptr_t)b.q[l] | (uintptr_t)b.k[l]) & 15u) != 0) return RTK_E_ALIGN;
        if ((b.q_stride_h[l] | b.q_stride_l[l] | b.k_stride_h[l] | b.k_stride_l[l]) % 8 != 0) return RTK_E_ALIGN;
    }
    if (workspace_bytes < rtk_pivot_score_workspace_bytes(b.H * b.n, b.L)) return RTK_E_WORKSPACE;

    ScoreParams prm;
    prm.H = (int)(b.H * b.n);
    prm.Hl = (int)b.H;
    prm.G = (int)(b.H / b.KVH);
    prm.L = (int)b.L;
    prm.nt = (int)((b.L + kTile - 1) / kTile);
    prm.n_atoms = (int)(b.D / 64);
    prm.q_dim1_is_l = prm.k_dim1_is_l = prm.kc_dim1_is_l = 0;
    prm.n_keys = b.n_keys;
    if (b.n_keys)
        for (int l = 0; l < b.n; ++l)
            if (!b.kc[l] || !b.slot[l] || ((uintptr_t)b.kc[l] & 15u) != 0) return RTK_E_BADARG;
    const float sq = (float)sqrt((double)b.D);
    prm.inv_sqrt_d = 1.0f / sq;
    const size_t plane = (size_t)prm.H * prm.nt * kTile;
    prm.ml_part = reinterpret_cast<float2*>(workspace);
    prm.stats = reinterpret_cast<float*>(workspace) + 6 * plane;
    prm.colsum_part = prm.stats + plane;
    return b.n == 1 ? score_launch<1>(b, prm, st) : score_launch<kMaxBatchLayers>(b, prm, st);
}

}

extern "C" int rtk_pivot_score(const void* q, int64_t H, int64_t q_stride_h, int64_t q_stride_l, const void* k, int64_t KVH,
                               int64_t k_stride_h, int64_t k_stride_l, int64_t L, int64_t D, void* head_scores,
                               void* workspace, size_t workspace_bytes, void* stream) {
    RTK_NVTX("rtk_pivot_score");
    if (!q || !k || !head_scores || !workspace || H < 1 || KVH < 1 || L < 1) return RTK_E_BADARG;
    ScoreBatch b = {};
    b.n = 1; b.H = H; b.KVH = KVH; b.L = L; b.D = D;
    b.q[0] = q; b.k[0] = k; b.head_scores[0] = head_scores;
    b.q_stride_h[0] = q_stride_h; b.q_stride_l[0] = q_stride_l; b.k_stride_h[0] = k_stride_h; b.k_stride_l[0] = k_stride_l;
    return pivot_score_batch(b, workspace, workspace_bytes, (cudaStream_t)stream);
}
```

### video-retake_b200/csrc/rtk_common.cuh

```cuda
#pragma once

#include <cuda_bf16.h>
#include <cuda_runtime.h>
#include <nvtx3/nvToolsExt.h>
#include <stdint.h>

#include "../../include/rtk_b200.h"

namespace rtk {

extern long long g_launches;

#define RTK_CHECK_LAUNCH()                                   \
    do {                                                     \
        ++::rtk::g_launches;                                 \
        cudaError_t e__ = cudaGetLastError();                \
        if (e__ != cudaSuccess) return (int)e__;             \
    } while (0)

constexpr int kWarp = 32;

struct NvtxRange {
    explicit NvtxRange(const char* name) { nvtxRangePushA(name); }
    ~NvtxRange() { nvtxRangePop(); }
    NvtxRange(const NvtxRange&) = delete;
    NvtxRange& operator=(const NvtxRange&) = delete;
};
#define RTK_NVTX(name) ::rtk::NvtxRange nvtx_range__(name)

struct DisAux {
    float* sim;
    float* nrm;
    long long si, sp;
};
int dpselect_sim_nrm(const void* x, int64_t T, int64_t N, int64_t C, DisAux aux, cudaStream_t st);

constexpr int kMaxBatchLayers = 32;
struct ScoreBatch {
    int n;
    int64_t H, KVH, L, D;
    const void* q[kMaxBatchLayers];
    const void* k[kMaxBatchLayers];
    void* head_scores[kMaxBatchLayers];
    int64_t q_stride_h[kMaxBatchLayers], q_stride_l[kMaxBatchLayers], k_stride_h[kMaxBatchLayers], k_stride_l[kMaxBatchLayers];
    const void* kc[kMaxBatchLayers];
    const int32_t* slot[kMaxBatchLayers];
    const int32_t* n_keys;
};
int pivot_score_batch(const ScoreBatch& b, void* workspace, size_t workspace_bytes, cudaStream_t st);

__device__ __forceinline__ void pdl_trigger() { asm volatile("griddepcontrol.launch_dependents;" ::: "memory"); }
__device__ __forceinline__ void pdl_wait() { asm volatile("griddepcontrol.wait;" ::: "memory"); }
#ifndef RTK_PDL_EARLY_SMALL
#define RTK_PDL_EARLY_SMALL 1
#endif
#ifndef RTK_PDL_EARLY_SCORE
#define RTK_PDL_EARLY_SCORE 1
#endif
__device__ __forceinline__ void pdl_enter() {
    if (RTK_PDL_EARLY_SMALL) pdl_trigger();
    pdl_wait();
}

bool pdl_enabled();

template <typename... KArgs, typename... Args>
static inline cudaError_t launch_pdl(void (*kern)(KArgs...), dim3 grid, dim3 block, size_t smem, cudaStream_t st,
                                     Args&&... args) {
    cudaLaunchConfig_t cfg = {};
    cfg.gridDim = grid;
    cfg.blockDim = block;
    cfg.dynamicSmemBytes = smem;
    cfg.stream = st;
    cudaLaunchAttribute attr[1];
    attr[0].id = cudaLaunchAttributeProgrammaticStreamSerialization;
    attr[0].val.programmaticStreamSerializationAllowed = 1;
    cfg.attrs = attr;
    cfg.numAttrs = pdl_enabled() ? 1 : 0;
    return cudaLaunchKernelEx(&cfg, kern, static_cast<KArgs>(args)...);
}
#define RTK_LAUNCH_PDL(kern, grid, block, smem, st, ...)                                                  \
    do {                                                                                                  \
        ++::rtk::g_launches;                                                                              \
        cudaError_t le__ = ::rtk::launch_pdl(kern, dim3(grid), dim3(block), (size_t)(smem), st, __VA_ARGS__); \
        if (le__ != cudaSuccess) return (int)le__;                                                        \
    } while (0)

__device__ __forceinline__ float bf16lo_to_f32(uint32_t packed) { return __uint_as_float(packed << 16); }
__device__ __forceinline__ float bf16hi_to_f32(uint32_t packed) { return __uint_as_float(packed & 0xffff0000u); }

__device__ __forceinline__ uint32_t pack_bf16x2_rn(float lo, float hi) {
    uint32_t d;
    asm("cvt.rn.bf16x2.f32 %0, %1, %2;" : "=r"(d) : "f"(hi), "f"(lo));
    return d;
}
__device__ __forceinline__ float round_bf16(float x) {
    return __bfloat162float(__float2bfloat16_rn(x));
}
__device__ __forceinline__ uint32_t mul_bf16x2_rn(uint32_t a, uint32_t b) {
    uint32_t d;
    asm("mul.rn.bf16x2 %0, %1, %2;" : "=r"(d) : "r"(a), "r"(b));
    return d;
}

__device__ __forceinline__ void fma_sq_bf16x2(float& acc_lo, float& acc_hi, uint32_t p) {
    asm("{\n\t.reg .b16 lo, hi;\n\t"
        "mov.b32 {lo, hi}, %2;\n\t"
        "fma.rn.f32.bf16 %0, lo, lo, %0;\n\t"
        "fma.rn.f32.bf16 %1, hi, hi, %1;\n\t}"
        : "+f"(acc_lo), "+f"(acc_hi)
        : "r"(p));
}
__device__ __forceinline__ void add_bf16x2(float& acc_lo, float& acc_hi, uint32_t p) {
    asm("{\n\t.reg .b16 lo, hi;\n\t"
        "mov.b32 {lo, hi}, %2;\n\t"
        "add.rn.f32.bf16 %0, lo, %0;\n\t"
        "add.rn.f32.bf16 %1, hi, %1;\n\t}"
        : "+f"(acc_lo), "+f"(acc_hi)
        : "r"(p));
}
__device__ __forceinline__ uint32_t scale_bf16x2_rn(uint32_t p, float s) {
    return pack_bf16x2_rn(bf16lo_to_f32(p) * s, bf16hi_to_f32(p) * s);
}

__device__ __forceinline__ uint32_t f32_to_ordered(float v) {
    uint32_t x = __float_as_uint(v);
    uint32_t mask = (x & 0x80000000u) ? 0xffffffffu : 0x80000000u;
    return (v == v) ? (x ^ mask) : 0xffffffffu;
}

__device__ __forceinline__ uint32_t smem_u32(const void* p) { return (uint32_t)__cvta_generic_to_shared(p); }

__device__ __forceinline__ void mbar_init(uint32_t bar, uint32_t count) {
    asm volatile("mbarrier.init.shared::cta.b64 [%0], %1;" ::"r"(bar), "r"(count) : "memory");
}
__device__ __forceinline__ void fence_mbar_init() {
    asm volatile("fence.mbarrier_init.release.cluster;" ::: "memory");
}
__device__ __forceinline__ void fence_proxy_async() {
    asm volatile("fence.proxy.async.shared::cta;" ::: "memory");
}
__device__ __forceinline__ void mbar_arrive_expect_tx(uint32_t bar, uint32_t bytes) {
    asm volatile("mbarrier.arrive.expect_tx.shared::cta.b64 _, [%0], %1;" ::"r"(bar), "r"(bytes) : "memory");
}
__device__ __forceinline__ void mbar_arrive(uint32_t bar) {
    asm volatile("mbarrier.arrive.shared::cta.b64 _, [%0];" ::"r"(bar) : "memory");
}
__device__ __forceinline__ bool mbar_try_wait(uint32_t bar, uint32_t parity) {
    uint32_t ok;
    asm volatile(
        "{\n\t.reg .pred p;\n\t"
        "mbarrier.try_wait.parity.shared::cta.b64 p, [%1], %2;\n\t"
        "selp.u32 %0, 1, 0, p;\n\t}"
        : "=r"(ok)
        : "r"(bar), "r"(parity)
        : "memory");
    return ok != 0;
}
__device__ __forceinline__ void mbar_wait(uint32_t bar, uint32_t parity) {
    while (!mbar_try_wait(bar, parity)) {
    }
}
__device__ __forceinline__ void bulk_g2s(uint32_t dst_smem, const void* src, uint32_t bytes, uint32_t bar) {
    asm volatile("cp.async.bulk.shared::cluster.global.mbarrier::complete_tx::bytes [%0], [%1], %2, [%3];" ::"r"(dst_smem),
                 "l"(src), "r"(bytes), "r"(bar)
                 : "memory");
}
__device__ __forceinline__ void bulk_s2g(void* dst, uint32_t src_smem, uint32_t bytes) {
    asm volatile("cp.async.bulk.global.shared::cta.bulk_group [%0], [%1], %2;" ::"l"(dst), "r"(src_smem), "r"(bytes)
                 : "memory");
}
__device__ __forceinline__ void bulk_commit() { asm volatile("cp.async.bulk.commit_group;" ::: "memory"); }
template <int N>
__device__ __forceinline__ void bulk_wait_read() {
    asm volatile("cp.async.bulk.wait_group.read %0;" ::"n"(N) : "memory");
}
template <int N>
__device__ __forceinline__ void bulk_wait_all() {
    asm volatile("cp.async.bulk.wait_group %0;" ::"n"(N) : "memory");
}

__device__ __forceinline__ bool elect_one() {
    uint32_t pred;
    asm volatile(
        "{\n\t.reg .pred p;\n\t"
        "elect.sync _|p, 0xffffffff;\n\t"
        "selp.u32 %0, 1, 0, p;\n\t}"
        : "=r"(pred));
    return pred != 0;
}

}
```

Measured before the change: 3598.

## Fuse Q un-RoPE into score kernel and fold key compaction into K un-RoPE

Drops the standalone Q+K un-RoPE pass. Q is now TMA-loaded raw into the score kernel, where dedicated rotation warps un-rotate it in shared memory using a precomputed cos/sin table, and the unroped Q is written back via TMA store for later passes. A new K-only un-RoPE kernel builds that cos/sin table and writes compacted keys directly into the elided key cache, replacing the separate keys-compact gather. This removes a full HBM round trip of Q and one kernel launch, at the cost of extra warps, barriers and complexity in the score kernel plus workspace for the rope tables.

```diff
diff --git a/video-retake_b200/csrc/pivot_misc.cu b/video-retake_b200/csrc/pivot_misc.cu
--- a/video-retake_b200/csrc/pivot_misc.cu
+++ b/video-retake_b200/csrc/pivot_misc.cu
@@ -73,102 +73,7 @@
     si = __bfloat162float(__float2bfloat16_rn(sinf(ang) * scaling));
 }
 
-#ifndef RTK_UNROPE_TOK
-#define RTK_UNROPE_TOK 2
-#endif
-constexpr int kUnropeTok = RTK_UNROPE_TOK;
-
-__device__ __forceinline__ uint32_t sub_bf16x2_rn(uint32_t a, uint32_t b) {
-    uint32_t d;
-    asm("sub.rn.bf16x2 %0, %1, %2;" : "=r"(d) : "r"(a), "r"(b));
-    return d;
-}
-__device__ __forceinline__ uint32_t add_bf16x2_rn(uint32_t a, uint32_t b) {
-    uint32_t d;
-    asm("add.rn.bf16x2 %0, %1, %2;" : "=r"(d) : "r"(a), "r"(b));
-    return d;
-}
-__device__ __forceinline__ void unrotate_bf16x2(uint32_t xa, uint32_t xb, uint32_t cs, uint32_t sn, bool scale, float inv_scale2,
-                                                uint32_t& oa, uint32_t& ob) {
-    const uint32_t ta = mul_bf16x2_rn(xa, cs), ra = mul_bf16x2_rn(xb ^ 0x80008000u, sn);
-    const uint32_t tb = mul_bf16x2_rn(xb, cs), rb = mul_bf16x2_rn(xa, sn);
-    oa = sub_bf16x2_rn(ta, ra);
-    ob = sub_bf16x2_rn(tb, rb);
-    if (scale) {
-        oa = scale_bf16x2_rn(oa, inv_scale2);
-        ob = scale_bf16x2_rn(ob, inv_scale2);
-    }
-}
-
-__device__ __forceinline__ void unrope_qk_body(const __nv_bfloat16* __restrict__ x, const long long* __restrict__ pos,
-                                               const float* __restrict__ inv_freq, float scaling,
-                                               __nv_bfloat16* __restrict__ out, const RopeParams& p) {
-    __shared__ __align__(16) __nv_bfloat16 s_cos[kUnropeTok][128], s_sin[kUnropeTok][128];
-    const int half = p.D >> 1;
-    const int vec_per_row = half >> 3;
-    const int ntask = (p.heads + p.heads2) * vec_per_row;
-    const int tid = threadIdx.x;
-    const bool scale = p.inv_scale2 != 1.0f;
-    const int v0 = tid % vec_per_row, h0 = tid / vec_per_row;
-    const bool second0 = h0 >= p.heads;
-    const long long src_h0 = second0 ? (long long)(h0 - p.heads) * p.stride_h2 : (long long)h0 * p.stride_h;
-    const long long src_l0 = second0 ? p.stride_l2 : p.stride_l;
-    const __nv_bfloat16* src0 = (second0 ? p.x2 : x) + src_h0 + v0 * 8;
-    for (int l0 = blockIdx.x * kUnropeTok; l0 < p.L; l0 += gridDim.x * kUnropeTok) {
-        const int nl = min(kUnropeTok, p.L - l0);
-        uint4 lo4[kUnropeTok], hi4[kUnropeTok];
-        if (tid < ntask) {
-#pragma unroll
-            for (int t = 0; t < kUnropeTok; ++t) {
-                if (t < nl) {
-                    lo4[t] = *reinterpret_cast<const uint4*>(src0 + (l0 + t) * src_l0);
-                    hi4[t] = *reinterpret_cast<const uint4*>(src0 + (l0 + t) * src_l0 + half);
-                }
-            }
-        }
-        for (int e = tid; e < nl * half; e += blockDim.x) {
-            const int t = e / half, c = e - t * half;
-            long long pv[3] = {0, 0, 0};
-            for (int r = 0; r < p.n_pos; ++r) pv[r] = pos[(size_t)r * p.L + l0 + t];
-            float co, si;
-            rope_table_entry(p, inv_freq, pv, c, scaling, co, si);
-            s_cos[t][c] = __float2bfloat16_rn(co);
-            s_sin[t][c] = __float2bfloat16_rn(si);
-        }
-        __syncthreads();
-#pragma unroll
-        for (int t = 0; t < kUnropeTok; ++t) {
-            if (t >= nl) break;
-            const int l = l0 + t;
-            for (int task = tid; task < ntask; task += blockDim.x) {
-                const int v = task % vec_per_row, h = task / vec_per_row;
-                const int c0 = v * 8;
-                const bool second = h >= p.heads;
-                const __nv_bfloat16* src = second ? p.x2 + (h - p.heads) * p.stride_h2 + l * p.stride_l2 : x + h * p.stride_h + l * p.stride_l;
-                __nv_bfloat16* dst = second ? p.out2 + (h - p.heads) * p.out_stride_h2 + l * p.out_stride_l2
-                                            : out + h * p.out_stride_h + l * p.out_stride_l;
-                uint4 a4 = lo4[t], b4 = hi4[t];
-                if (task != tid) {
-                    a4 = *reinterpret_cast<const uint4*>(src + c0);
-                    b4 = *reinterpret_cast<const uint4*>(src + c0 + half);
-                }
-                const uint4 cs = *reinterpret_cast<const uint4*>(&s_cos[t][c0]);
-                const uint4 sn = *reinterpret_cast<const uint4*>(&s_sin[t][c0]);
-                uint4 ol4, oh4;
-                unrotate_bf16x2(a4.x, b4.x, cs.x, sn.x, scale, p.inv_scale2, ol4.x, oh4.x);
-                unrotate_bf16x2(a4.y, b4.y, cs.y, sn.y, scale, p.inv_scale2, ol4.y, oh4.y);
-                unrotate_bf16x2(a4.z, b4.z, cs.z, sn.z, scale, p.inv_scale2, ol4.z, oh4.z);
-                unrotate_bf16x2(a4.w, b4.w, cs.w, sn.w, scale, p.inv_scale2, ol4.w, oh4.w);
-                *reinterpret_cast<uint4*>(dst + c0) = ol4;
-                *reinterpret_cast<uint4*>(dst + c0 + half) = oh4;
-            }
-        }
-        __syncthreads();
-    }
-}
-
 struct BatchLayers {
-    const __nv_bfloat16* q[kMaxBatchLayers];
     const __nv_bfloat16* k[kMaxBatchLayers];
     const __nv_bfloat16* k_in[kMaxBatchLayers];
     const __nv_bfloat16* v[kMaxBatchLayers];
@@ -181,22 +86,11 @@
     long long* pos_out[kMaxBatchLayers];
     int32_t* keep_idx[kMaxBatchLayers];
     const __nv_bfloat16* head_scores[kMaxBatchLayers];
-    long long q_stride_h[kMaxBatchLayers], q_stride_l[kMaxBatchLayers];
     long long kin_stride_h[kMaxBatchLayers], kin_stride_l[kMaxBatchLayers];
     long long k_stride_h[kMaxBatchLayers], k_stride_l[kMaxBatchLayers];
     long long v_stride_h[kMaxBatchLayers], v_stride_l[kMaxBatchLayers];
     long long out_stride_h[kMaxBatchLayers], pos_out_stride[kMaxBatchLayers];
 };
-
-__global__ void __launch_bounds__(256)
-pivot_unrope_qk_batch_kernel(const __grid_constant__ BatchLayers t, const float* __restrict__ inv_freq, float scaling, RopeParams p) {
-    pdl_enter();
-    const int layer = blockIdx.y;
-    p.stride_h = t.q_stride_h[layer]; p.stride_l = t.q_stride_l[layer];
-    p.x2 = t.k_in[layer]; p.out2 = t.ku[layer];
-    p.stride_h2 = t.kin_stride_h[layer]; p.stride_l2 = t.kin_stride_l[layer];
-    unrope_qk_body(t.q[layer], t.pos[layer], inv_freq, scaling, t.qu[layer], p);
-}
 
 __global__ void __launch_bounds__(256)
 pivot_rope_kernel(const __nv_bfloat16* __restrict__ x, const __nv_bfloat16* __restrict__ cos_t,
@@ -300,6 +194,75 @@
     for (int i = beg; i < end; ++i) slot[i] = (m && m[i]) ? -1 : base++;
 }
 
+constexpr int kUnropeKThreads = 256;
+__global__ void __launch_bounds__(kUnropeKThreads)
+pivot_unrope_k_batch_kernel(const __grid_constant__ BatchLayers t, const __grid_constant__ KeyElide e, int elide,
+                            const float* __restrict__ inv_freq, float scaling, RopeParams p, __nv_bfloat16* __restrict__ cos_t,
+                            __nv_bfloat16* __restrict__ sin_t) {
+    pdl_enter();
+    __shared__ __align__(16) __nv_bfloat16 s_cos[kUnropeKThreads], s_sin[kUnropeKThreads];
+    const int layer = blockIdx.y, tid = threadIdx.x;
+    const int half = p.D >> 1, vpr = half >> 3;
+    const int ntok = kUnropeKThreads / half;
+    const int l0 = blockIdx.x * ntok;
+    const int ntask = ntok * p.heads2 * vpr;
+    const bool scale = p.inv_scale2 != 1.0f;
+    const __nv_bfloat16* __restrict__ k = t.k_in[layer];
+    const long long sh = t.kin_stride_h[layer], sl = t.kin_stride_l[layer];
+    uint4 lo0 = {}, hi0 = {};
+    if (tid < ntask) {
+        const int v = tid % vpr, h = (tid / vpr) % p.heads2, l = l0 + tid / (vpr * p.heads2);
+        if (l < p.L) {
+            lo0 = *reinterpret_cast<const uint4*>(k + h * sh + l * sl + v * 8);
+            hi0 = *reinterpret_cast<const uint4*>(k + h * sh + l * sl + v * 8 + half);
+        }
+    }
+    {
+        const int l = l0 + tid / half, c = tid % half;
+        if (l < p.L) {
+            const long long* pos = t.pos[layer];
+            long long pv[3] = {0, 0, 0};
+            for (int r = 0; r < p.n_pos; ++r) pv[r] = pos[(size_t)r * p.L + l];
+            float co, si;
+            rope_table_entry(p, inv_freq, pv, c, scaling, co, si);
+            s_cos[tid] = __float2bfloat16_rn(co);
+            s_sin[tid] = __float2bfloat16_rn(si);
+            const size_t o = ((size_t)layer * p.L + l) * half + c;
+            cos_t[o] = s_cos[tid];
+            sin_t[o] = s_sin[tid];
+        }
+    }
+    __syncthreads();
+    for (int task = tid; task < ntask; task += kUnropeKThreads) {
+        const int v = task % vpr, h = (task / vpr) % p.heads2, tk = task / (vpr * p.heads2);
+        const int l = l0 + tk, c0 = v * 8;
+        if (l >= p.L) continue;
+        uint4 a4 = lo0, b4 = hi0;
+        if (task != tid) {
+            a4 = *reinterpret_cast<const uint4*>(k + h * sh + l * sl + c0);
+            b4 = *reinterpret_cast<const uint4*>(k + h * sh + l * sl + c0 + half);
+        }
+        const uint4 cs = *reinterpret_cast<const uint4*>(&s_cos[tk * half + c0]);
+        const uint4 sn = *reinterpret_cast<const uint4*>(&s_sin[tk * half + c0]);
+        uint4 ol4, oh4;
+        unrotate_bf16x2(a4.x, b4.x, cs.x, sn.x, scale, p.inv_scale2, ol4.x, oh4.x);
+        unrotate_bf16x2(a4.y, b4.y, cs.y, sn.y, scale, p.inv_scale2, ol4.y, oh4.y);
+        unrotate_bf16x2(a4.z, b4.z, cs.z, sn.z, scale, p.inv_scale2, ol4.z, oh4.z);
+        unrotate_bf16x2(a4.w, b4.w, cs.w, sn.w, scale, p.inv_scale2, ol4.w, oh4.w);
+        __nv_bfloat16* dst = t.ku[layer] + h * p.out_stride_h2 + l * p.out_stride_l2;
+        *reinterpret_cast<uint4*>(dst + c0) = ol4;
+        *reinterpret_cast<uint4*>(dst + c0 + half) = oh4;
+        if (elide) {
+            const int s = e.slot[layer][l];
+            if (s >= 0) {
+                __nv_bfloat16* kc = e.kc[layer] + ((size_t)s * e.KVH + h) * e.D;
+                *reinterpret_cast<uint4*>(kc + c0) = ol4;
+                *reinterpret_cast<uint4*>(kc + c0 + half) = oh4;
+            }
+        }
+    }
+}
+
 __global__ void __launch_bounds__(256)
 pivot_keys_compact_kernel(const __grid_constant__ KeyElide e) {
     pdl_enter();
@@ -319,12 +282,13 @@
     }
 }
 
-static int key_elide_prepare(KeyElide& ke, int n, ScoreBatch& sb, cudaStream_t st) {
-    RTK_LAUNCH_PDL(pivot_keymask_scan_kernel, (unsigned)n, 1024, 0, st, ke);
-    const long long total = (long long)ke.L * ke.KVH * (ke.D >> 3);
-    long long gx = (total + 255) / 256;
-    if (gx > 148 * 8) gx = 148 * 8;
-    RTK_LAUNCH_PDL(pivot_keys_compact_kernel, dim3((unsigned)gx, (unsigned)n), 256, 0, st, ke);
+static int key_elide_prepare(KeyElide& ke, int n, ScoreBatch& sb, bool gather, cudaStream_t st) {
+    if (gather) {
+        const long long total = (long long)ke.L * ke.KVH * (ke.D >> 3);
+        long long gx = (total + 255) / 256;
+        if (gx > 148 * 8) gx = 148 * 8;
+        RTK_LAUNCH_PDL(pivot_keys_compact_kernel, dim3((unsigned)gx, (unsigned)n), 256, 0, st, ke);
+    }
     for (int i = 0; i < n; ++i) {
         sb.kc[i] = ke.kc[i];
         sb.slot[i] = ke.slot[i];
@@ -807,7 +771,7 @@
     const size_t n = (size_t)(n_layers < kMaxBatchLayers ? n_layers : kMaxBatchLayers);
     return align256(rtk_pivot_score_workspace_bytes(H * (int64_t)n, L)) +
            n * (align256((size_t)H * L * D * 2) + align256((size_t)KVH * L * D * 2)) + align256(n * sizeof(long long)) + 256 +
-           n * key_elide_bytes(KVH, L, D) + 256;
+           2 * align256(n * L * (D / 2) * 2) + n * key_elide_bytes(KVH, L, D) + 256;
 }
 
 extern "C" size_t rtk_pivot_update_workspace_bytes(int64_t H, int64_t KVH, int64_t L, int64_t D) {
@@ -828,6 +792,9 @@
     char* qu0 = ws;                     ws += (size_t)n * align256((size_t)H * L * D * 2);
     char* ku0 = ws;                     ws += (size_t)n * align256((size_t)KVH * L * D * 2);
     long long* tmin = (long long*)ws;   ws += align256((size_t)n * sizeof(long long)) + 256;
+    const size_t rope_bytes = align256((size_t)n * L * (D / 2) * 2);
+    __nv_bfloat16* rope_cos = (__nv_bfloat16*)ws;  ws += rope_bytes;
+    __nv_bfloat16* rope_sin = (__nv_bfloat16*)ws;  ws += rope_bytes;
     char* kc0 = ws;                     ws += (size_t)n * align256((size_t)KVH * L * D * 2);
     char* slot0 = ws;                   ws += (size_t)n * align256((size_t)L * 4);
     int32_t* nkeys_ws = (int32_t*)ws;
@@ -839,7 +806,6 @@
         const rtk_pivot_update_args& x = a[i < n ? i : 0];
         char* qu = qu0 + (size_t)(i < n ? i : 0) * align256((size_t)H * L * D * 2);
         char* ku = ku0 + (size_t)(i < n ? i : 0) * align256((size_t)KVH * L * D * 2);
-        t.q[i] = (const __nv_bfloat16*)x.q;       t.q_stride_h[i] = x.q_stride_h;     t.q_stride_l[i] = x.q_stride_l;
         t.k_in[i] = (const __nv_bfloat16*)x.k;    t.kin_stride_h[i] = x.k_stride_h;   t.kin_stride_l[i] = x.k_stride_l;
         t.qu[i] = (__nv_bfloat16*)qu;             t.ku[i] = (__nv_bfloat16*)ku;
         t.k[i] = reforge ? (const __nv_bfloat16*)ku : (const __nv_bfloat16*)x.k;
@@ -867,31 +833,38 @@
     mrope_bounds(a0.n_pos, a0.mrope_section, D, rp.bound);
     const bool xchg = a0.xchg_world > 1;
     const int64_t score_rows = a0.score_rows > 0 ? a0.score_rows : KVH;
-    if (reforge && !a0.skip_score) {
-        if (a0.inv_freq) {
-            RTK_LAUNCH_PDL(pivot_unrope_qk_batch_kernel, dim3((unsigned)((L + kUnropeTok - 1) / kUnropeTok), (unsigned)n), 256, 0, st, t, a0.inv_freq,
-                           a0.attention_scaling, rp);
-        } else {
+    if (!a0.skip_score) {
+        const bool unrope_in_score = reforge && a0.inv_freq;
+        bool any_mask = false;
+        for (int i = 0; i < n; ++i) any_mask = any_mask || a[i].keymask != nullptr;
+        const bool elide = any_mask && key_elision_enabled();
+        KeyElide ke = {};
+        ke.L = (int)L; ke.KVH = (int)KVH; ke.D = (int)D; ke.n_keys = nkeys_ws;
+        for (int i = 0; i < kMaxBatchLayers; ++i) {
+            const int j = i < n ? i : 0;
+            ke.keymask[i] = a[j].keymask;
+            ke.slot[i] = (int32_t*)(slot0 + (size_t)j * align256((size_t)L * 4));
+            ke.k[i] = t.k[j]; ke.k_stride_h[i] = t.k_stride_h[j]; ke.k_stride_l[i] = t.k_stride_l[j];
+            ke.kc[i] = (__nv_bfloat16*)(kc0 + (size_t)j * align256((size_t)KVH * L * D * 2));
+        }
+        if (elide) RTK_LAUNCH_PDL(pivot_keymask_scan_kernel, (unsigned)n, 1024, 0, st, ke);
+        if (unrope_in_score) {
+            const int ntok = kUnropeKThreads / (int)(D / 2);
+            RTK_LAUNCH_PDL(pivot_unrope_k_batch_kernel, dim3((unsigned)((L + ntok - 1) / ntok), (unsigned)n), kUnropeKThreads, 0, st,
+                           t, ke, elide ? 1 : 0, a0.inv_freq, a0.attention_scaling, rp, rope_cos, rope_sin);
+            sb.unrope = 1;
+            sb.rope_cos = rope_cos; sb.rope_sin = rope_sin; sb.inv_scale2 = a0.inv_scale2;
+            for (int i = 0; i < n; ++i) {
+                sb.qr[i] = a[i].q; sb.qr_stride_h[i] = a[i].q_stride_h; sb.qr_stride_l[i] = a[i].q_stride_l;
+            }
+        } else if (reforge) {
             rp.stride_h = a0.q_stride_h; rp.stride_l = a0.q_stride_l;
             rp.x2 = t.k_in[0]; rp.out2 = t.ku[0]; rp.stride_h2 = a0.k_stride_h; rp.stride_l2 = a0.k_stride_l;
             const int rc = rope_launch(a0.q, a0.cos, a0.sin, t.qu[0], rp, st);
             if (rc) return rc;
         }
-    }
-    if (!a0.skip_score) {
-        bool any_mask = false;
-        for (int i = 0; i < n; ++i) any_mask = any_mask || a[i].keymask != nullptr;
-        if (any_mask && key_elision_enabled()) {
-            KeyElide ke = {};
-            ke.L = (int)L; ke.KVH = (int)KVH; ke.D = (int)D; ke.n_keys = nkeys_ws;
-            for (int i = 0; i < kMaxBatchLayers; ++i) {
-                const int j = i < n ? i : 0;
-                ke.keymask[i] = a[j].keymask;
-                ke.slot[i] = (int32_t*)(slot0 + (size_t)j * align256((size_t)L * 4));
-                ke.k[i] = t.k[j]; ke.k_stride_h[i] = t.k_stride_h[j]; ke.k_stride_l[i] = t.k_stride_l[j];
-                ke.kc[i] = (__nv_bfloat16*)(kc0 + (size_t)j * align256((size_t)KVH * L * D * 2));
-            }
-            int rc = key_elide_prepare(ke, n, sb, st);
+        if (elide) {
+            int rc = key_elide_prepare(ke, n, sb, !unrope_in_score, st);
             if (rc) return rc;
         }
         if (a0.ev_score_begin) cudaEventRecord((cudaEvent_t)a0.ev_score_begin, st);
diff --git a/video-retake_b200/csrc/pivot_score.cu b/video-retake_b200/csrc/pivot_score.cu
--- a/video-retake_b200/csrc/pivot_score.cu
+++ b/video-retake_b200/csrc/pivot_score.cu
@@ -20,7 +20,7 @@
     static constexpr uint32_t stats = b_ring + kStages * kTileBytes;
     static constexpr uint32_t merge = stats + kStatSlots * kTile * 4;
     static constexpr uint32_t bars = merge + 4 * kTile * 2 * 4;
-    static constexpr uint32_t n_bars = 4 + 2 * kStages + 2 * kAccBufs + kStatSlots;
+    static constexpr uint32_t n_bars = 4 + 2 * kStages + 2 * kAccBufs + kStatSlots + 2;
     static constexpr uint32_t tmem_ptr = bars + n_bars * 8;
     static constexpr uint32_t total = tmem_ptr + 16;
 };
@@ -79,6 +79,11 @@
         ::"r"(dst), "l"(reinterpret_cast<uint64_t>(map)), "r"(bar), "r"(c0), "r"(c1), "r"(c2)
         : "memory");
 }
+__device__ __forceinline__ void tma_store_3d(const CUtensorMap* map, uint32_t src, int c0, int c1, int c2) {
+    asm volatile("cp.async.bulk.tensor.3d.global.shared::cta.bulk_group [%0, {%2, %3, %4}], [%1];"
+                 ::"l"(reinterpret_cast<uint64_t>(map)), "r"(src), "r"(c0), "r"(c1), "r"(c2)
+                 : "memory");
+}
 __device__ __forceinline__ float ex2f(float x) {
     float y;
     asm("ex2.approx.ftz.f32 %0, %1;" : "=f"(y) : "f"(x));
@@ -100,6 +105,7 @@
 struct ScoreMaps {
     CUtensorMap q[NL], k[NL];
     CUtensorMap kc[NL];
+    CUtensorMap qr[NL];
 };
 
 struct ScoreParams {
@@ -113,6 +119,10 @@
     float2* ml_part;
     float* stats;
     float* colsum_part;
+    int unrope, qr_dim1_is_l;
+    const __nv_bfloat16* rope_cos;
+    const __nv_bfloat16* rope_sin;
+    float inv_scale2;
 };
 
 constexpr float kLog2e = 1.4426950408889634f;
@@ -251,13 +261,52 @@
     }
 };
 
+constexpr int kRotPer = 2;
+struct RotSlice {
+    uint4 cs[kRotPer], sn[kRotPer];
+    __device__ __forceinline__ void load(int i0, int total, int lg_cpr, int half, int row0, int L, const __nv_bfloat16* cos_l,
+                                         const __nv_bfloat16* sin_l, int lane) {
+#pragma unroll
+        for (int u = 0; u < kRotPer; ++u) {
+            const int i = i0 + lane + 32 * u, j = i & ((1 << lg_cpr) - 1), l = row0 + (i >> lg_cpr);
+            if (i < total && l < L) {
+                cs[u] = __ldg(reinterpret_cast<const uint4*>(cos_l + (size_t)l * half + j * 8));
+                sn[u] = __ldg(reinterpret_cast<const uint4*>(sin_l + (size_t)l * half + j * 8));
+            }
+        }
+    }
+    __device__ __forceinline__ void rotate(uint8_t* pair, int i0, int total, int lg_cpr, int n_atoms, int row0, int L,
+                                           float inv_scale2, int lane) const {
+        const bool scale = inv_scale2 != 1.0f;
+#pragma unroll
+        for (int u = 0; u < kRotPer; ++u) {
+            const int i = i0 + lane + 32 * u, j = i & ((1 << lg_cpr) - 1), rr = i >> lg_cpr;
+            if (i >= total || row0 + rr >= L) continue;
+            const int r = rr & (kTile - 1);
+            const uint32_t lo = (uint32_t)(rr >> 7) * kTileBytes + r * 128 + ((j ^ (r & 7)) << 4);
+            const uint32_t hi = n_atoms == 2 ? lo + kHalfBytes : lo ^ 64u;
+            const uint4 a4 = *reinterpret_cast<const uint4*>(pair + lo), b4 = *reinterpret_cast<const uint4*>(pair + hi);
+            uint4 ol4, oh4;
+            unrotate_bf16x2(a4.x, b4.x, cs[u].x, sn[u].x, scale, inv_scale2, ol4.x, oh4.x);
+            unrotate_bf16x2(a4.y, b4.y, cs[u].y, sn[u].y, scale, inv_scale2, ol4.y, oh4.y);
+            unrotate_bf16x2(a4.z, b4.z, cs[u].z, sn[u].z, scale, inv_scale2, ol4.z, oh4.z);
+            unrotate_bf16x2(a4.w, b4.w, cs[u].w, sn[u].w, scale, inv_scale2, ol4.w, oh4.w);
+            *reinterpret_cast<uint4*>(pair + lo) = ol4;
+            *reinterpret_cast<uint4*>(pair + hi) = oh4;
+        }
+    }
+};
+
 constexpr int kGroups = 4;
 constexpr int kSoftmaxWarps = 4 * kGroups;
+constexpr int kRotWarp0 = 2 + kSoftmaxWarps;
+constexpr int kRotWarps = 2;
 constexpr int kScoreThreads2 = (2 + kSoftmaxWarps) * 32;
+constexpr int kScoreThreads1 = kScoreThreads2 + kRotWarps * 32;
 constexpr int kTileArrivals = 8;
 
 template <int PASS, int NL>
-__global__ void __launch_bounds__(kScoreThreads2, 1)
+__global__ void __launch_bounds__(PASS == 1 ? kScoreThreads1 : kScoreThreads2, 1)
 pivot_score_kernel(const __grid_constant__ ScoreMaps<NL> maps, ScoreParams prm) {
     if (RTK_PDL_EARLY_SCORE) pdl_trigger();
     extern __shared__ __align__(1024) uint8_t smem_raw[];
@@ -273,9 +322,14 @@
     auto t_full = [&](int b) { return bar0 + 32 + 8 * (2 * kStages + b); };
     auto t_empty = [&](int b) { return bar0 + 32 + 8 * (2 * kStages + kAccBufs + b); };
     auto st_full = [&](int i) { return bar0 + 32 + 8 * (2 * kStages + 2 * kAccBufs + i); };
+    auto a_raw = [&](int i) { return bar0 + 32 + 8 * (2 * kStages + 2 * kAccBufs + kStatSlots + i); };
 
     if (threadIdx.x == 0) {
-        for (int i = 0; i < 2; ++i) { mbar_init(a_full(i), 1); mbar_init(a_empty(i), 1); }
+        for (int i = 0; i < 2; ++i) {
+            mbar_init(a_full(i), (PASS == 1 && prm.unrope) ? kRotWarps : 1);
+            mbar_init(a_empty(i), 1);
+            mbar_init(a_raw(i), 1);
+        }
         for (int s = 0; s < kStages; ++s) { mbar_init(b_full(s), 1); mbar_init(b_empty(s), 1); }
         for (int b = 0; b < kAccBufs; ++b) { mbar_init(t_full(b), 1); mbar_init(t_empty(b), kTileArrivals); }
         for (int i = 0; i < kStatSlots; ++i) mbar_init(st_full(i), 1);
@@ -299,7 +353,66 @@
     int ul, tb0, tb1;
 
     if (warp == 0) {
-        if (lane == 0) {
+        if (PASS == 1 && prm.unrope) {
+            if (lane == 0) {
+                TileRange ra = range;
+                uint32_t cnt = 0, acnt = 0;
+                int p_as = 0, p_layer = 0, p_head = 0, p_row0 = 0, p_npa = 0;
+                uint32_t p_par = 0;
+                bool p_store = false;
+                auto issue_pair = [&]() {
+                    int aul, atb0, atb1;
+                    if (!ra.next(aul, atb0, atb1)) return;
+                    const int h = aul / ra.nta, ta = (aul - h * ra.nta) * kPair;
+                    p_as = acnt % kASlots; p_layer = ra.layer; p_head = h; p_row0 = ta * kTile;
+                    p_npa = (ta + 1 < ra.nt_a) ? 2 : 1;
+                    p_par = (acnt / kASlots) & 1u;
+                    p_store = atb0 == 0;
+                    mbar_wait_feeder(a_empty(p_as), p_par ^ 1u);
+                    bulk_wait_read<1>();
+                    mbar_arrive_expect_tx(a_raw(p_as), p_npa * prm.n_atoms * kHalfBytes);
+                    const int l1 = prm.qr_dim1_is_l;
+                    for (int pa = 0; pa < p_npa; ++pa)
+                        for (int kk = 0; kk < prm.n_atoms; ++kk) {
+                            const int row = p_row0 + pa * kTile;
+                            tma_load_3d(base + ScoreSmem::a_tile + (p_as * kPair + pa) * kTileBytes + kk * kHalfBytes,
+                                        maps.qr + p_layer, kk * 64, l1 ? row : h, l1 ? h : row, a_raw(p_as));
+                        }
+                    ++acnt;
+                };
+                issue_pair();
+                while (range.next(ul, tb0, tb1)) {
+                    const int layer = range.layer;
+                    const int b_head = (ul / range.nta) / prm.G;
+                    const CUtensorMap* b_map = maps.k + layer;
+                    const int b_l1 = prm.k_dim1_is_l;
+                    for (int tb = tb0; tb < tb1; ++tb, ++cnt) {
+                        const int s = cnt % kStages;
+                        mbar_wait_feeder(b_empty(s), ((cnt / kStages) & 1u) ^ 1u);
+                        mbar_arrive_expect_tx(b_full(s), prm.n_atoms * kHalfBytes);
+                        const uint32_t dst = base + ScoreSmem::b_ring + s * kTileBytes;
+                        for (int kk = 0; kk < prm.n_atoms; ++kk) {
+                            const int row = tb * kTile;
+                            tma_load_3d(dst + kk * kHalfBytes, b_map, kk * 64, b_l1 ? row : b_head, b_l1 ? b_head : row, b_full(s));
+                        }
+                        if (tb != tb0) continue;
+                        mbar_wait_feeder(a_full(p_as), p_par);
+                        if (p_store) {
+                            const int l1 = prm.q_dim1_is_l;
+                            for (int pa = 0; pa < p_npa; ++pa)
+                                for (int kk = 0; kk < prm.n_atoms; ++kk) {
+                                    const int row = p_row0 + pa * kTile;
+                                    tma_store_3d(maps.q + p_layer, base + ScoreSmem::a_tile + (p_as * kPair + pa) * kTileBytes + kk * kHalfBytes,
+                                                 kk * 64, l1 ? row : p_head, l1 ? p_head : row);
+                                }
+                        }
+                        bulk_commit();
+                        issue_pair();
+                    }
+                }
+                bulk_wait_all<0>();
+            }
+        } else if (lane == 0) {
             uint32_t cnt = 0, ucnt = 0;
             while (range.next(ul, tb0, tb1)) {
                 const int layer = range.layer;
@@ -369,6 +482,35 @@
                     if (tb == tb1 - 1) tc_commit(a_empty(as));
                 }
                 __syncwarp();
+            }
+        }
+    } else if (warp >= kRotWarp0) {
+        if (PASS == 1 && prm.unrope) {
+            const int w = warp - kRotWarp0;
+            const int lg_cpr = prm.n_atoms == 2 ? 3 : 2;
+            const int half = prm.n_atoms * 32;
+            uint32_t acnt = 0;
+            while (range.next(ul, tb0, tb1)) {
+                const int h = ul / range.nta, ta = (ul - h * range.nta) * kPair;
+                const int as = acnt % kASlots;
+                const int total = ((ta + 1 < range.nt_a) ? 2 : 1) * kTile << lg_cpr;
+                const int i0 = (total / 32) * w / kRotWarps * 32, i1 = (total / 32) * (w + 1) / kRotWarps * 32;
+                const size_t tab = (size_t)range.layer * prm.L * half;
+                uint8_t* pair = smem + ScoreSmem::a_tile + as * kPair * kTileBytes;
+                RotSlice sl;
+                sl.load(i0, i1, lg_cpr, half, ta * kTile, prm.L, prm.rope_cos + tab, prm.rope_sin + tab, lane);
+                mbar_wait(a_raw(as), (acnt / kASlots) & 1u);
+                for (int i = i0; i < i1; i += 32 * kRotPer) {
+                    RotSlice nx;
+                    if (i + 32 * kRotPer < i1)
+                        nx.load(i + 32 * kRotPer, i1, lg_cpr, half, ta * kTile, prm.L, prm.rope_cos + tab, prm.rope_sin + tab, lane);
+                    sl.rotate(pair, i, i1, lg_cpr, prm.n_atoms, ta * kTile, prm.L, prm.inv_scale2, lane);
+                    sl = nx;
+                }
+                fence_proxy_async();
+                __syncwarp();
+                if (lane == 0) mbar_arrive(a_full(as));
+                ++acnt;
             }
         }
     } else {
@@ -551,6 +693,15 @@
         if (rc) return rc;
         if (l == 0) { prm.q_dim1_is_l = ql; prm.k_dim1_is_l = kl; }
         else if (ql != prm.q_dim1_is_l || kl != prm.k_dim1_is_l) return RTK_E_UNSUPPORTED;
+        if (prm.unrope) {
+            int rl = 0;
+            rc = make_map(&maps.qr[l], b.qr[l], b.H, b.L, b.D, b.qr_stride_h[l], b.qr_stride_l[l], &rl);
+            if (rc) return rc;
+            if (l == 0) prm.qr_dim1_is_l = rl;
+            else if (rl != prm.qr_dim1_is_l) return RTK_E_UNSUPPORTED;
+        } else {
+            maps.qr[l] = maps.q[l];
+        }
         if (prm.n_keys) {
             int cl = 0;
             rc = make_map(&maps.kc[l], b.kc[l], b.KVH, b.L, b.D, b.D, b.KVH * b.D, &cl);
@@ -560,7 +711,7 @@
             maps.kc[l] = maps.k[l];
         }
     }
-    for (int l = b.n; l < NL; ++l) { maps.q[l] = maps.q[0]; maps.k[l] = maps.k[0]; maps.kc[l] = maps.kc[0]; }
+    for (int l = b.n; l < NL; ++l) { maps.q[l] = maps.q[0]; maps.k[l] = maps.k[0]; maps.kc[l] = maps.kc[0]; maps.qr[l] = maps.qr[0]; }
     int dev = 0, sms = 0;
     cudaGetDevice(&dev);
     cudaDeviceGetAttribute(&sms, cudaDevAttrMultiProcessorCount, dev);
@@ -578,7 +729,7 @@
         out.p[l] = reinterpret_cast<__nv_bfloat16*>(b.head_scores[l < b.n ? l : 0]);
         out.slot[l] = prm.n_keys ? b.slot[l < b.n ? l : 0] : nullptr;
     }
-    RTK_LAUNCH_PDL((pivot_score_kernel<1, NL>), grid, kScoreThreads2, smem, st, maps, prm);
+    RTK_LAUNCH_PDL((pivot_score_kernel<1, NL>), grid, kScoreThreads1, smem, st, maps, prm);
     dim3 g1((unsigned)((prm.nt * kTile + 255) / 256), (unsigned)prm.H);
     RTK_LAUNCH_PDL(pivot_stats_merge_kernel, g1, 256, 0, st, prm.ml_part, prm.H, prm.L, prm.nt * kTile, prm.stats);
     RTK_LAUNCH_PDL((pivot_score_kernel<2, NL>), grid, kScoreThreads2, smem, st, maps, prm);
@@ -610,6 +761,18 @@
     if (b.n_keys)
         for (int l = 0; l < b.n; ++l)
             if (!b.kc[l] || !b.slot[l] || ((uintptr_t)b.kc[l] & 15u) != 0) return RTK_E_BADARG;
+    prm.unrope = b.unrope ? 1 : 0;
+    prm.qr_dim1_is_l = 0;
+    prm.rope_cos = b.rope_cos;
+    prm.rope_sin = b.rope_sin;
+    prm.inv_scale2 = b.inv_scale2;
+    if (b.unrope) {
+        if (!b.rope_cos || !b.rope_sin || (((uintptr_t)b.rope_cos | (uintptr_t)b.rope_sin) & 15u) != 0) return RTK_E_BADARG;
+        for (int l = 0; l < b.n; ++l) {
+            if (!b.qr[l]) return RTK_E_BADARG;
+            if (((uintptr_t)b.qr[l] & 15u) != 0 || (b.qr_stride_h[l] | b.qr_stride_l[l]) % 8 != 0) return RTK_E_ALIGN;
+        }
+    }
     const float sq = (float)sqrt((double)b.D);
     prm.inv_sqrt_d = 1.0f / sq;
     const size_t plane = (size_t)prm.H * prm.nt * kTile;
diff --git a/video-retake_b200/csrc/rtk_common.cuh b/video-retake_b200/csrc/rtk_common.cuh
--- a/video-retake_b200/csrc/rtk_common.cuh
+++ b/video-retake_b200/csrc/rtk_common.cuh
@@ -46,6 +46,12 @@
     const void* kc[kMaxBatchLayers];
     const int32_t* slot[kMaxBatchLayers];
     const int32_t* n_keys;
+    int unrope;
+    const void* qr[kMaxBatchLayers];
+    int64_t qr_stride_h[kMaxBatchLayers], qr_stride_l[kMaxBatchLayers];
+    const __nv_bfloat16* rope_cos;
+    const __nv_bfloat16* rope_sin;
+    float inv_scale2;
 };
 int pivot_score_batch(const ScoreBatch& b, void* workspace, size_t workspace_bytes, cudaStream_t st);
 
@@ -123,6 +129,23 @@
     return pack_bf16x2_rn(bf16lo_to_f32(p) * s, bf16hi_to_f32(p) * s);
 }
 
+__device__ __forceinline__ uint32_t sub_bf16x2_rn(uint32_t a, uint32_t b) {
+    uint32_t d;
+    asm("sub.rn.bf16x2 %0, %1, %2;" : "=r"(d) : "r"(a), "r"(b));
+    return d;
+}
+__device__ __forceinline__ void unrotate_bf16x2(uint32_t xa, uint32_t xb, uint32_t cs, uint32_t sn, bool scale, float inv_scale2,
+                                                uint32_t& oa, uint32_t& ob) {
+    const uint32_t ta = mul_bf16x2_rn(xa, cs), ra = mul_bf16x2_rn(xb ^ 0x80008000u, sn);
+    const uint32_t tb = mul_bf16x2_rn(xb, cs), rb = mul_bf16x2_rn(xa, sn);
+    oa = sub_bf16x2_rn(ta, ra);
+    ob = sub_bf16x2_rn(tb, rb);
+    if (scale) {
+        oa = scale_bf16x2_rn(oa, inv_scale2);
+        ob = scale_bf16x2_rn(ob, inv_scale2);
+    }
+}
+
 __device__ __forceinline__ uint32_t f32_to_ordered(float v) {
     uint32_t x = __float_as_uint(v);
     uint32_t mask = (x & 0x80000000u) ? 0xffffffffu : 0x80000000u;
```

After: 3625 (median of 6 runs). No clear change (+0.8%).
